# vibevoice-community/VibeVoice

Measured on NVIDIA H100. Metric: audio_seconds_per_second, higher is better.
Workload: dtype bf16

## Files before the change

### include/vibevoice_b200.h

```cpp
#ifndef VIBEVOICE_B200_H_
#define VIBEVOICE_B200_H_

#include <stdint.h>

#ifdef __cplusplus
extern "C" {
#endif

#define VV_ABI_VERSION 1

typedef struct vv_ctx vv_ctx;

typedef enum {
  VV_OK = 0,
  VV_ERR_INVALID = -1,
  VV_ERR_CUDA = -2,
  VV_ERR_STATE = -3,
  VV_ERR_NOMEM = -4
} vv_status;

typedef enum { VV_DT_BF16 = 0, VV_DT_F32 = 1, VV_DT_F16 = 2 } vv_dtype;

typedef struct {
  int32_t hidden_size, intermediate_size, num_layers, num_q_heads, num_kv_heads, head_dim, vocab_size;
  int32_t max_position_embeddings, tie_word_embeddings;
  float rms_norm_eps, rope_theta;
  int32_t head_layers, head_ffn_dim, latent_size;
  float head_rms_eps;
  int32_t n_stages;
  int32_t dec_ratios[8];
  int32_t dec_depths[8];
  int32_t dec_n_filters;
  int32_t enc_ratios[8];
  int32_t enc_depths[8];
  int32_t enc_n_filters;
  int32_t acoustic_vae_dim, semantic_vae_dim;
  float codec_eps;
  int32_t n_valid_ids;
  int32_t valid_ids[8];
  int32_t max_batch;
  int32_t max_diffusion_steps;
} vv_model_desc;

int vv_abi_version(void);
const char* vv_last_error(void);
int vv_create(const vv_model_desc* desc, int device, vv_ctx** out);
void vv_destroy(vv_ctx* ctx);

int vv_load_tensor(vv_ctx* ctx, const char* name, const void* data, int dtype, const int64_t* shape, int ndim);
int vv_set_speech_factors(vv_ctx* ctx, float scaling_factor, float bias_factor);
int vv_finalize_weights(vv_ctx* ctx);
int64_t vv_weight_bytes(vv_ctx* ctx, int which);

int vv_kv_init(vv_ctx* ctx, int64_t n_pages);
int vv_kv_reserve(vv_ctx* ctx, int seq, int64_t n_tokens, void* stream);
int vv_kv_set_len(vv_ctx* ctx, int seq, int64_t len, void* stream);
int vv_kv_write(vv_ctx* ctx, int seq, int layer, int64_t pos0, int64_t n_tokens,
                const void* k_bf16, const void* v_bf16, void* stream);
int vv_kv_delete_slot(vv_ctx* ctx, int seq, int64_t pos, void* stream);
int64_t vv_kv_pages_free(vv_ctx* ctx);
int64_t vv_kv_pages_total(vv_ctx* ctx);

int vv_set_rope_inv_freq(vv_ctx* ctx, const float* inv_freq_host, int n);
int vv_set_row_mode(vv_ctx* ctx, const int32_t* row_mode_host, void* stream);
int vv_lm_decode(vv_ctx* ctx, const float* embeds, float* hidden, float* logits, int32_t* tokens, void* stream);
int vv_lm_head(vv_ctx* ctx, const float* hidden , float* logits, int32_t* tokens, void* stream);
int vv_lm_logits_full(vv_ctx* ctx, const float* hidden , float* logits_out, void* stream);
int vv_lm_decode_range(vv_ctx* ctx, const float* embeds, int layer_begin, int layer_end, int final_norm, float* hidden, void* stream);
int vv_kv_commit(vv_ctx* ctx, const int32_t* advance_host, void* stream);
int64_t vv_kv_len(vv_ctx* ctx, int seq);
int vv_embed_tokens(vv_ctx* ctx, const int32_t* tokens_host, int n, float* out , void* stream);

int vv_set_diffusion_steps(vv_ctx* ctx, int n_steps, const float* timesteps, const float* coef, void* stream);
int vv_set_diffusion_steps_sde(vv_ctx* ctx, int n_steps, const float* timesteps, const float* coef7, void* stream);
int vv_set_step_noise(vv_ctx* ctx, const float* step_noise);
int vv_diffusion_sample(vv_ctx* ctx, const float* cond, const float* noise, const int32_t* active, float cfg_scale,
                        float* latent_out, void* stream);

int vv_codec_decode_frame(vv_ctx* ctx, const float* latent, const int32_t* active, float* audio_out , void* stream);
int vv_semantic_encode_frame(vv_ctx* ctx, const float* audio , const int32_t* active, float* feat_out , void* stream);
int vv_connect(vv_ctx* ctx, const float* latent , const float* sem , const int32_t* active,
               float* embeds_inout , void* stream);
int vv_codec_state_zero(vv_ctx* ctx, const int32_t* rows_host, int n, void* stream);
int vv_codec_state_reset(vv_ctx* ctx, void* stream);

int vv_frame_tail(vv_ctx* ctx, const float* hidden, const float* noise, const int32_t* active, float cfg_scale,
                  float* latent_out, float* audio_out, float* embeds_inout, void* stream);

int64_t vv_launch_count(vv_ctx* ctx);
int vv_debug_gemv(vv_ctx* ctx, const void* w_bf16, const float* bias, const float* x, float* y, int M, int N, int K,
                  int prologue, const float* pro_w, float eps, int epilogue, void* stream);

int vv_debug_barrier_bench(vv_ctx* ctx, int iters, int ctas_per_sm, float* ms_out);
int vv_debug_stream_gemv(vv_ctx* ctx, const void* w_bf16, const float* bias, const float* x, float* y, int M, int N, int K, int prologue,
                         const float* pro_w, float eps, int alpha_kind, const float* alpha, int accumulate, void* stream);
int vv_debug_stream_gemv2(vv_ctx* ctx, const void* w_bf16, const float* bias, const float* x, int64_t ldx, float* y, int64_t ldy, int M, int N,
                          int K, int prologue, const float* pro_w, float eps, const float* pro_shift, const float* pro_scale, int64_t pro_ld,
                          int alpha_kind, const float* alpha, int64_t lda, int store, int64_t operand_cap, void* stream);
int vv_stream_trace_read2(vv_ctx* ctx, long long* out , int max_ops);
int vv_stream_trace_read(vv_ctx* ctx, long long* out , int* out_meta , int max_ops, const char* program_prefix);
int vv_stream_diag(vv_ctx* ctx, unsigned* out6);

#ifdef __cplusplus
}
#endif
#endif
```

### vibevoice_b200/_native.py

```python
from __future__ import annotations

import ctypes as C
import os
from typing import Optional, Sequence

import numpy as np

_HERE = os.path.dirname(os.path.abspath(__file__))
LIB_PATH = os.path.join(_HERE, "csrc", "libvibevoice_b200.so")

VV_DT_BF16, VV_DT_F32, VV_DT_F16 = 0, 1, 2
PRO_NONE, PRO_RMSNORM, PRO_ADALN, PRO_SILU = 0, 1, 2, 3
EPI_NONE, EPI_RESID, EPI_GATED_RESID, EPI_GAMMA_RESID, EPI_SWIGLU, EPI_GELU, EPI_SILU = 0, 2, 3, 4, 5, 6, 7


class VVError(RuntimeError):
    pass


class ModelDesc(C.Structure):
    _fields_ = [
        ("hidden_size", C.c_int32), ("intermediate_size", C.c_int32), ("num_layers", C.c_int32),
        ("num_q_heads", C.c_int32), ("num_kv_heads", C.c_int32), ("head_dim", C.c_int32), ("vocab_size", C.c_int32),
        ("max_position_embeddings", C.c_int32), ("tie_word_embeddings", C.c_int32),
        ("rms_norm_eps", C.c_float), ("rope_theta", C.c_float),
        ("head_layers", C.c_int32), ("head_ffn_dim", C.c_int32), ("latent_size", C.c_int32), ("head_rms_eps", C.c_float),
        ("n_stages", C.c_int32), ("dec_ratios", C.c_int32 * 8), ("dec_depths", C.c_int32 * 8), ("dec_n_filters", C.c_int32),
        ("enc_ratios", C.c_int32 * 8), ("enc_depths", C.c_int32 * 8), ("enc_n_filters", C.c_int32),
        ("acoustic_vae_dim", C.c_int32), ("semantic_vae_dim", C.c_int32), ("codec_eps", C.c_float),
        ("n_valid_ids", C.c_int32), ("valid_ids", C.c_int32 * 8),
        ("max_batch", C.c_int32), ("max_diffusion_steps", C.c_int32),
    ]


_P, _I, _L, _F = C.c_void_p, C.c_int, C.c_int64, C.c_float
SYMBOLS = {
    "vv_abi_version": (_I, []),
    "vv_last_error": (C.c_char_p, []),
    "vv_create": (_I, [C.POINTER(ModelDesc), _I, C.POINTER(_P)]),
    "vv_destroy": (None, [_P]),
    "vv_load_tensor": (_I, [_P, C.c_char_p, _P, _I, C.POINTER(_L), _I]),
    "vv_set_speech_factors": (_I, [_P, _F, _F]),
    "vv_finalize_weights": (_I, [_P]),
    "vv_weight_bytes": (_L, [_P, _I]),
    "vv_kv_init": (_I, [_P, _L]),
    "vv_kv_reserve": (_I, [_P, _I, _L, _P]),
    "vv_kv_set_len": (_I, [_P, _I, _L, _P]),
    "vv_kv_write": (_I, [_P, _I, _I, _L, _L, _P, _P, _P]),
    "vv_kv_delete_slot": (_I, [_P, _I, _L, _P]),
    "vv_kv_pages_free": (_L, [_P]),
    "vv_kv_pages_total": (_L, [_P]),
    "vv_set_rope_inv_freq": (_I, [_P, _P, _I]),
    "vv_set_row_mode": (_I, [_P, _P, _P]),
    "vv_lm_decode": (_I, [_P, _P, _P, _P, _P, _P]),
    "vv_lm_head": (_I, [_P, _P, _P, _P, _P]),
    "vv_lm_logits_full": (_I, [_P, _P, _P, _P]),
    "vv_lm_decode_range": (_I, [_P, _P, _I, _I, _I, _P, _P]),
    "vv_kv_commit": (_I, [_P, _P, _P]),
    "vv_kv_len": (_L, [_P, _I]),
    "vv_embed_tokens": (_I, [_P, _P, _I, _P, _P]),
    "vv_set_diffusion_steps": (_I, [_P, _I, _P, _P, _P]),
    "vv_set_diffusion_steps_sde": (_I, [_P, _I, _P, _P, _P]),
    "vv_set_step_noise": (_I, [_P, _P]),
    "vv_diffusion_sample": (_I, [_P, _P, _P, _P, _F, _P, _P]),
    "vv_codec_decode_frame": (_I, [_P, _P, _P, _P, _P]),
    "vv_semantic_encode_frame": (_I, [_P, _P, _P, _P, _P]),
    "vv_connect": (_I, [_P, _P, _P, _P, _P, _P]),
    "vv_codec_state_zero": (_I, [_P, _P, _I, _P]),
    "vv_codec_state_reset": (_I, [_P, _P]),
    "vv_frame_tail": (_I, [_P, _P, _P, _P, _F, _P, _P, _P, _P]),
    "vv_launch_count": (_L, [_P]),
    "vv_debug_barrier_bench": (_I, [_P, _I, _I, C.POINTER(C.c_float)]),
    "vv_debug_gemv": (_I, [_P, _P, _P, _P, _P, _I, _I, _I, _I, _P, _F, _I, _P]),
    "vv_debug_stream_gemv": (_I, [_P, _P, _P, _P, _P, _I, _I, _I, _I, _P, _F, _I, _P, _I, _P]),
    "vv_debug_stream_gemv2": (_I, [_P, _P, _P, _P, _L, _P, _L, _I, _I, _I, _I, _P, _F, _P, _P, _L, _I, _P, _L, _I, _L, _P]),
    "vv_stream_diag": (_I, [_P, _P]),
    "vv_stream_trace_read": (_I, [_P, _P, _P, _I, C.c_char_p]),
    "vv_stream_trace_read2": (_I, [_P, _P, _I]),
}

_lib = None


def load_library(path: Optional[str] = None):
    global _lib
    if _lib is not None and path is None:
        return _lib
    p = path or LIB_PATH
    if not os.path.exists(p):
        raise VVError("libvibevoice_b200.so not built (%s). Run `python -c 'import __graft_entry__ as g; g.build()'`; "
                      "there is no CPU fallback." % p)
    lib = C.CDLL(p)
    for name, (res, args) in SYMBOLS.items():
        fn = getattr(lib, name)
        fn.restype, fn.argtypes = res, args
    if path is None:
        _lib = lib
    return lib


def check(rc: int, what: str = ""):
    if rc < 0:
        msg = load_library().vv_last_error().decode("utf-8", "replace")
        raise VVError("%s failed (%d): %s" % (what or "vibevoice_b200 call", rc, msg))
    return rc


def iptr(a: np.ndarray):
    return a.ctypes.data_as(C.c_void_p)


def i32(seq: Sequence[int]) -> np.ndarray:
    return np.ascontiguousarray(np.asarray(seq, dtype=np.int32))
```

### vibevoice_b200/csrc/vv_kernels.cuh

```cuda
#pragma once
#include <cuda_bf16.h>
#include <cuda_runtime.h>
#include <stdint.h>

#define VV_DEVINL __device__ __forceinline__

namespace vv {

typedef __nv_bfloat16 bf16;

enum Prologue { PRO_NONE = 0, PRO_RMSNORM = 1, PRO_ADALN = 2, PRO_SILU = 3 };
enum Epilogue { EPI_NONE = 0, EPI_RESID = 2, EPI_GATED_RESID = 3, EPI_GAMMA_RESID = 4, EPI_SWIGLU = 5, EPI_GELU = 6, EPI_SILU = 7 };

struct RowMap {
  int T;
  long long bs;
  long long rs;
  VV_DEVINL long long off(int m) const { return (long long)(m / T) * bs + (long long)(m % T) * rs; }
};

static inline RowMap dense_rows(long long ld) { RowMap r; r.T = 1 << 30; r.bs = 0; r.rs = ld; return r; }

struct GemvP {
  const bf16* W;
  const float* bias;
  const float* x;
  RowMap xmap;
  float* y;
  int ldy;
  int M, N, K;
  int pro;
  const float* pro_w;
  float pro_eps;
  const float* pro_shift;
  const float* pro_scale;
  long long pro_ld;
  int epi;
  const float* epi_a;
  long long epi_lda;
  const float* res;
  int ldres;
  int WK;
};

VV_DEVINL void pdl_trigger() { asm volatile("griddepcontrol.launch_dependents;" ::: "memory"); }
VV_DEVINL void pdl_wait() { asm volatile("griddepcontrol.wait;" ::: "memory"); }

VV_DEVINL float warp_sum(float v) {
#pragma unroll
  for (int o = 16; o > 0; o >>= 1) v += __shfl_xor_sync(0xffffffffu, v, o);
  return v;
}
VV_DEVINL float warp_max(float v) {
#pragma unroll
  for (int o = 16; o > 0; o >>= 1) v = fmaxf(v, __shfl_xor_sync(0xffffffffu, v, o));
  return v;
}
VV_DEVINL float silu_f(float x) { return x / (1.0f + __expf(-x)); }
VV_DEVINL float gelu_erf_f(float x) { return 0.5f * x * (1.0f + erff(x * 0.70710678118654752440f)); }

VV_DEVINL uint4 ldg_stream(const void* p) {
  uint4 r;
  asm volatile("ld.global.nc.L1::no_allocate.v4.u32 {%0,%1,%2,%3}, [%4];"
               : "=r"(r.x), "=r"(r.y), "=r"(r.z), "=r"(r.w) : "l"(p));
  return r;
}
VV_DEVINL void bf16x8_unpack(const uint4& u, float* f) {
  f[0] = __uint_as_float(u.x << 16); f[1] = __uint_as_float(u.x & 0xffff0000u);
  f[2] = __uint_as_float(u.y << 16); f[3] = __uint_as_float(u.y & 0xffff0000u);
  f[4] = __uint_as_float(u.z << 16); f[5] = __uint_as_float(u.z & 0xffff0000u);
  f[6] = __uint_as_float(u.w << 16); f[7] = __uint_as_float(u.w & 0xffff0000u);
}
VV_DEVINL float bf16_bits_to_f(unsigned short b) { return __uint_as_float(((unsigned)b) << 16); }

VV_DEVINL int xs_pos(int k) {
  int c = k >> 8, kk = k & 255;
  int lane = kk >> 3, j = kk & 7;
  return (c << 8) + ((j >> 2) << 7) + (lane << 2) + (j & 3);
}

VV_DEVINL void epi_store_e(const GemvP& p, int epi, int m, int n, float v) {
  switch (epi) {
    case EPI_RESID: v += p.res[(long long)m * p.ldres + n]; break;
    case EPI_GATED_RESID: v = p.res[(long long)m * p.ldres + n] + p.epi_a[(long long)m * p.epi_lda + n] * v; break;
    case EPI_GAMMA_RESID: v = p.res[(long long)m * p.ldres + n] + p.epi_a[n] * v; break;
    case EPI_GELU: v = gelu_erf_f(v); break;
    case EPI_SILU: v = silu_f(v); break;
    default: break;
  }
  p.y[(long long)m * p.ldy + n] = v;
}
VV_DEVINL void epi_store(const GemvP& p, int m, int n, float v) { epi_store_e(p, p.epi, m, n, v); }

template <int MB>
__global__ void __launch_bounds__(256) gemv_kernel(GemvP p) {
  extern __shared__ __align__(16) float smem_f[];
  const int K = p.K, N = p.N;
  const int Kp = (K + 255) & ~255;
  float* xs = smem_f;
  float* red = smem_f + MB * Kp;
  __shared__ float s_part[MB][8];
  const int tid = threadIdx.x, lane = tid & 31, warp = tid >> 5;
  const int WK = p.WK, WR = 8 / WK;
  const int wr = warp / WK, wk = warp % WK;
  const int ntasks = (N + 4 * WR - 1) / (4 * WR);
  const int nchunks = (K + 255) >> 8;
  const int klane = lane * 8;

  auto load_chunk = [&](uint4 (&wv)[4], const bf16* const (&wrow)[4], int c) {
    if (c < nchunks && (c << 8) + klane < K) {
#pragma unroll
      for (int r = 0; r < 4; ++r) wv[r] = ldg_stream(wrow[r] + (c << 8));
    } else {
#pragma unroll
      for (int r = 0; r < 4; ++r) wv[r] = make_uint4(0u, 0u, 0u, 0u);
    }
  };
  auto set_rows = [&](const bf16* (&wrow)[4], int task) {
    const int r0 = (task * WR + wr) * 4;
#pragma unroll
    for (int r = 0; r < 4; ++r) wrow[r] = p.W + (size_t)min(r0 + r, N - 1) * K + klane;
  };

  pdl_trigger();
  for (int m0 = 0; m0 < p.M; m0 += MB) {
    __syncthreads();
    int task = blockIdx.x;
    const bf16* wrow[4];
    uint4 cur[4], nxt[4];
    int c = wk;
    if (task < ntasks) {
      set_rows(wrow, task);
      load_chunk(cur, wrow, c);
      load_chunk(nxt, wrow, c + WK);
    }
    pdl_wait();
    const bool need_inv = (p.pro == PRO_RMSNORM || p.pro == PRO_ADALN);
    const int K4 = K >> 2;
    constexpr int XR = 4;
    const bool one_pass = (K4 <= XR * 256);
    for (int m = 0; m < MB; ++m) {
      const bool valid = (m0 + m < p.M);
      const float* xr = p.x + (valid ? p.xmap.off(m0 + m) : 0);
      float4 xv[XR];
      float inv = 1.f;
      if (need_inv) {
        float ss = 0.f;
        if (one_pass) {
#pragma unroll
          for (int i = 0; i < XR; ++i) {
            const int q = tid + i * 256;
            xv[i] = (valid && q < K4) ? *reinterpret_cast<const float4*>(xr + 4 * q) : make_float4(0.f, 0.f, 0.f, 0.f);
            ss += xv[i].x * xv[i].x + xv[i].y * xv[i].y + xv[i].z * xv[i].z + xv[i].w * xv[i].w;
          }
        } else if (valid) {
          for (int q = tid; q < K4; q += 256) { const float4 v = *reinterpret_cast<const float4*>(xr + 4 * q); ss += v.x * v.x + v.y * v.y + v.z * v.z + v.w * v.w; }
        }
        ss = warp_sum(ss);
        if (lane == 0) s_part[m][warp] = ss;
        __syncthreads();
        float t = 0.f;
#pragma unroll
        for (int i = 0; i < 8; ++i) t += s_part[m][i];
        inv = rsqrtf(t / (float)K + p.pro_eps);
      }
      auto xform_store = [&](int k, float4 v, bool have) {
        if (valid && k < K) {
          if (!have) v = *reinterpret_cast<const float4*>(xr + k);
          if (p.pro == PRO_RMSNORM) {
            const float4 w = *reinterpret_cast<const float4*>(p.pro_w + k);
            v.x *= inv * w.x; v.y *= inv * w.y; v.z *= inv * w.z; v.w *= inv * w.w;
          } else if (p.pro == PRO_ADALN) {
            float4 w = make_float4(1.f, 1.f, 1.f, 1.f);
            if (p.pro_w) w = *reinterpret_cast<const float4*>(p.pro_w + k);
            const long long o = (long long)(m0 + m) * p.pro_ld + k;
            const float4 sc = *reinterpret_cast<const float4*>(p.pro_scale + o);
            const float4 sh = *reinterpret_cast<const float4*>(p.pro_shift + o);
            v.x = v.x * inv * w.x * (1.f + sc.x) + sh.x; v.y = v.y * inv * w.y * (1.f + sc.y) + sh.y;
            v.z = v.z * inv * w.z * (1.f + sc.z) + sh.z; v.w = v.w * inv * w.w * (1.f + sc.w) + sh.w;
          } else if (p.pro == PRO_SILU) {
            v.x = silu_f(v.x); v.y = silu_f(v.y); v.z = silu_f(v.z); v.w = silu_f(v.w);
          }
        } else {
          v = make_float4(0.f, 0.f, 0.f, 0.f);
        }
        *reinterpret_cast<float4*>(xs + m * Kp + xs_pos(k)) = v;
      };
#pragma unroll
      for (int i = 0; i < XR; ++i) {
        const int q = tid + i * 256;
        if (q < (Kp >> 2)) xform_store(q << 2, xv[i], need_inv && one_pass);
      }
      for (int q = tid + XR * 256; q < (Kp >> 2); q += 256) xform_store(q << 2, make_float4(0.f, 0.f, 0.f, 0.f), false);
    }
    __syncthreads();
// ... 421 lines not shown
               : "+f"(d[0]), "+f"(d[1]), "+f"(d[2]), "+f"(d[3]), "+f"(d[4]), "+f"(d[5]), "+f"(d[6]), "+f"(d[7]), "+f"(d[8]), "+f"(d[9]), "+f"(d[10]), "+f"(d[11]), "+f"(d[12]), "+f"(d[13]), "+f"(d[14]), "+f"(d[15]), "+f"(d[16]), "+f"(d[17]), "+f"(d[18]), "+f"(d[19]), "+f"(d[20]), "+f"(d[21]), "+f"(d[22]), "+f"(d[23]), "+f"(d[24]), "+f"(d[25]), "+f"(d[26]), "+f"(d[27]), "+f"(d[28]), "+f"(d[29]), "+f"(d[30]), "+f"(d[31])
               : "l"(a), "l"(b), "r"(accumulate) : "memory");
}

__global__ void split_bf16_kernel(const float* __restrict__ x, RowMap xmap, bf16* __restrict__ hi, bf16* __restrict__ lo, int M, int K) {
  pdl_trigger();
  pdl_wait();
  const long long n4 = (long long)M * (K >> 2);
  for (long long i = (long long)blockIdx.x * blockDim.x + threadIdx.x; i < n4; i += (long long)gridDim.x * blockDim.x) {
    const int m = (int)(i / (K >> 2)), k = (int)(i % (K >> 2)) << 2;
    const float4 v = *reinterpret_cast<const float4*>(x + xmap.off(m) + k);
    const float h0 = __bfloat162float(__float2bfloat16_rn(v.x)), h1 = __bfloat162float(__float2bfloat16_rn(v.y));
    const float h2 = __bfloat162float(__float2bfloat16_rn(v.z)), h3 = __bfloat162float(__float2bfloat16_rn(v.w));
    *reinterpret_cast<uint2*>(hi + (size_t)m * K + k) = make_uint2(pack_bf16(h0, h1), pack_bf16(h2, h3));
    *reinterpret_cast<uint2*>(lo + (size_t)m * K + k) = make_uint2(pack_bf16(v.x - h0, v.y - h1), pack_bf16(v.z - h2, v.w - h3));
  }
}

__global__ void __launch_bounds__(128) gemm_wgmma_kernel(GemvP p, const bf16* __restrict__ a_hi, const bf16* __restrict__ a_lo) {
  extern __shared__ unsigned char wg_raw[];
  const unsigned raw_addr = smem_u32(wg_raw);
  unsigned char* sm = wg_raw + ((1024u - (raw_addr & 1023u)) & 1023u);
  const int tid = threadIdx.x, lane = tid & 31, warp = tid >> 5;
  const int bn = blockIdx.x * WG_BM;
  const int bm = blockIdx.y * WG_BN;
  const int K = p.K, nk = (K + WG_BK - 1) / WG_BK;

  auto load_w = [&](int stage, int kb) {
    unsigned char* wt = sm + stage * WG_STAGE;
#pragma unroll
    for (int i = 0; i < 8; ++i) {
      const int idx = tid + i * 128, r = idx >> 3, c = idx & 7;
      const int n = bn + r, k = kb * WG_BK + c * 8;
      const bool ok = (n < p.N) && (k < K);
      cp_async16(wt + r * 128 + ((c ^ (r & 7)) << 4), p.W + (size_t)(ok ? n : 0) * K + (ok ? k : 0), ok ? 16 : 0);
    }
  };
  auto load_a = [&](int stage, int kb) {
    unsigned char* ah = sm + stage * WG_STAGE + WG_BM * 128;
#pragma unroll
    for (int i = 0; i < 8; ++i) {
      const int idx = tid + i * 128, pl = idx >> 9, r = (idx >> 3) & 63, c = idx & 7;
      const int m = bm + r, k = kb * WG_BK + c * 8;
      const bool ok = (m < p.M) && (k < K);
      const bf16* src = (pl ? a_lo : a_hi) + (size_t)(ok ? m : 0) * K + (ok ? k : 0);
      cp_async16(ah + pl * (WG_BN * 128) + r * 128 + ((c ^ (r & 7)) << 4), src, ok ? 16 : 0);
    }
  };
  float acc[2][32];
#pragma unroll
  for (int h = 0; h < 2; ++h)
#pragma unroll
    for (int i = 0; i < 32; ++i) acc[h][i] = 0.f;

  pdl_trigger();
  load_w(0, 0);
  if (nk > 1) load_w(1, 1);
  pdl_wait();
  load_a(0, 0);
  cp_async_commit();
  if (nk > 1) load_a(1, 1);
  cp_async_commit();
  for (int kb = 0; kb < nk; ++kb) {
    const int st = kb % WG_NST;
    cp_async_wait<1>();
    asm volatile("fence.proxy.async.shared::cta;" ::: "memory");
    __syncthreads();
    const unsigned wbase = smem_u32(sm + st * WG_STAGE);
    const unsigned long long dw = wgmma_desc_sw128(wbase), dh = wgmma_desc_sw128(wbase + WG_BM * 128),
                             dl = wgmma_desc_sw128(wbase + WG_BM * 128 + WG_BN * 128);
    wgmma_fence();
#pragma unroll
    for (int k = 0; k < WG_BK / 16; ++k) {
#pragma unroll
      for (int h = 0; h < 2; ++h) {
        wgmma_m64n64(acc[h], dw + 512 * h + 2 * k, dh + 2 * k, 1);
        wgmma_m64n64(acc[h], dw + 512 * h + 2 * k, dl + 2 * k, 1);
      }
    }
    wgmma_commit();
    if (kb + 2 < nk) {
      wgmma_wait<1>();
      __syncthreads();
      load_w((kb + 2) % WG_NST, kb + 2);
      load_a((kb + 2) % WG_NST, kb + 2);
    }
    cp_async_commit();
  }
  wgmma_wait<0>();
#pragma unroll
  for (int h = 0; h < 2; ++h)
#pragma unroll
    for (int e = 0; e < 2; ++e) {
      const int n = bn + h * 64 + warp * 16 + (lane >> 2) + 8 * e;
      if (n >= p.N) continue;
      const float bias = p.bias ? p.bias[n] : 0.f;
#pragma unroll
      for (int j = 0; j < WG_BN / 8; ++j)
#pragma unroll
        for (int c = 0; c < 2; ++c) {
          const int m = bm + 8 * j + 2 * (lane & 3) + c;
          if (m < p.M) epi_store(p, m, n, acc[h][4 * j + 2 * e + c] + bias);
        }
    }
}

__global__ void conv_naive_kernel(const float* __restrict__ W, const float* __restrict__ bias, const float* __restrict__ x,
                                  RowMap xmap, float* __restrict__ y, int M, int N, int K) {
  pdl_trigger();
  pdl_wait();
  const long long idx = (long long)blockIdx.x * blockDim.x + threadIdx.x;
  if (idx >= (long long)M * N) return;
  const int m = (int)(idx / N), n = (int)(idx % N);
  const float* xr = x + xmap.off(m);
  const float* wr = W + (size_t)n * K;
  float acc = bias ? bias[n] : 0.f;
  for (int k = 0; k < K; ++k) acc = fmaf(wr[k], xr[k], acc);
  y[idx] = acc;
}

__global__ void __launch_bounds__(256) conv_warp_kernel(const float* __restrict__ W, const float* __restrict__ bias, const float* __restrict__ x,
                                                        RowMap xmap, float* __restrict__ y, int M, int N, int K) {
  pdl_trigger();
  pdl_wait();
  const long long idx = (long long)blockIdx.x * (blockDim.x >> 5) + (threadIdx.x >> 5);
  const int lane = threadIdx.x & 31;
  if (idx >= (long long)M * N) return;
  const int m = (int)(idx / N), n = (int)(idx % N);
  const float* xr = x + xmap.off(m);
  const float* wr = W + (size_t)n * K;
  float acc = 0.f;
  for (int k = lane; k < K; k += 32) acc = fmaf(wr[k], xr[k], acc);
  acc = warp_sum(acc);
  if (lane == 0) y[idx] = acc + (bias ? bias[n] : 0.f);
}

__global__ void rows_norm_kernel(const float* __restrict__ x, const float* __restrict__ w, float* __restrict__ y,
                                 int M, int C, float eps) {
  pdl_trigger();
  pdl_wait();
  const int row = blockIdx.x * (blockDim.x >> 5) + (threadIdx.x >> 5);
  const int lane = threadIdx.x & 31;
  if (row >= M) return;
  const float* xr = x + (size_t)row * C;
  float ss = 0.f;
  for (int c = lane; c < C; c += 32) { float v = xr[c]; ss += v * v; }
  ss = warp_sum(ss);
  const float inv = rsqrtf(ss / (float)C + eps);
  for (int c = lane; c < C; c += 32) y[(size_t)row * C + c] = xr[c] * inv * (w ? w[c] : 1.f);
}

__global__ void assemble_window_kernel(const float* __restrict__ src, const float* __restrict__ hist,
                                       float* __restrict__ win, float* __restrict__ hist_next, int B, int T, int ctx, int C,
                                       const float* __restrict__ norm_w, float eps, float alpha, float beta) {
  pdl_trigger();
  pdl_wait();
  const int row = blockIdx.x * (blockDim.x >> 5) + (threadIdx.x >> 5);
  const int lane = threadIdx.x & 31;
  const int R = ctx + T;
  if (row >= B * R) return;
  const int b = row / R, j = row % R;
  float* wr = win + ((size_t)b * R + j) * C;
  float* hn = (j >= T) ? hist_next + ((size_t)b * ctx + (j - T)) * C : nullptr;
  if (j < ctx) {
    const float* hr = hist + ((size_t)b * ctx + j) * C;
    for (int c = lane; c < C; c += 32) { float v = hr[c]; wr[c] = v; if (hn) hn[c] = v; }
  } else {
    const float* sr = src + ((size_t)b * T + (j - ctx)) * C;
    float inv = 1.f;
    if (norm_w) {
      float ss = 0.f;
      for (int c = lane; c < C; c += 32) { float v = sr[c]; ss += v * v; }
      ss = warp_sum(ss);
      inv = rsqrtf(ss / (float)C + eps);
    }
    for (int c = lane; c < C; c += 32) {
      float v = norm_w ? sr[c] * inv * norm_w[c] : sr[c] * alpha + beta;
      wr[c] = v;
      if (hn) hn[c] = v;
    }
  }
}

__global__ void __launch_bounds__(256) assemble_window_block_kernel(const float* __restrict__ src, const float* __restrict__ hist,
                                                                    float* __restrict__ win, float* __restrict__ hist_next, int B, int T,
                                                                    int ctx, int C, const float* __restrict__ norm_w, float eps, float alpha,
                                                                    float beta) {
  pdl_trigger();
  pdl_wait();
  const int row = blockIdx.x, tid = threadIdx.x;
  const int R = ctx + T;
  const int b = row / R, j = row % R;
  float* wr = win + ((size_t)b * R + j) * C;
  float* hn = (j >= T) ? hist_next + ((size_t)b * ctx + (j - T)) * C : nullptr;
  __shared__ float sp[8];
  if (j < ctx) {
    const float* hr = hist + ((size_t)b * ctx + j) * C;
    for (int c = tid; c < C; c += 256) { float v = hr[c]; wr[c] = v; if (hn) hn[c] = v; }
  } else {
    const float* sr = src + ((size_t)b * T + (j - ctx)) * C;
    float inv = 1.f;
    if (norm_w) {
      float ss = 0.f;
      for (int c = tid; c < C; c += 256) { float v = sr[c]; ss += v * v; }
      ss = warp_sum(ss);
      if ((tid & 31) == 0) sp[tid >> 5] = ss;
      __syncthreads();
      float t = 0.f;
#pragma unroll
      for (int i = 0; i < 8; ++i) t += sp[i];
      inv = rsqrtf(t / (float)C + eps);
    }
    for (int c = tid; c < C; c += 256) {
      float v = norm_w ? sr[c] * inv * norm_w[c] : sr[c] * alpha + beta;
      wr[c] = v;
      if (hn) hn[c] = v;
    }
  }
}
__global__ void __launch_bounds__(256) rows_norm_block_kernel(const float* __restrict__ x, const float* __restrict__ w, float* __restrict__ y,
                                                              int C, float eps) {
  pdl_trigger();
  pdl_wait();
  const int row = blockIdx.x, tid = threadIdx.x;
  const float* xr = x + (size_t)row * C;
  __shared__ float sp[8];
  float ss = 0.f;
  for (int c = tid; c < C; c += 256) { float v = xr[c]; ss += v * v; }
  ss = warp_sum(ss);
  if ((tid & 31) == 0) sp[tid >> 5] = ss;
  __syncthreads();
  float t = 0.f;
#pragma unroll
  for (int i = 0; i < 8; ++i) t += sp[i];
  const float inv = rsqrtf(t / (float)C + eps);
  for (int c = tid; c < C; c += 256) y[(size_t)row * C + c] = xr[c] * inv * (w ? w[c] : 1.f);
}

__global__ void dwconv_res_kernel(const float* __restrict__ x, const float* __restrict__ win, const float* __restrict__ w ,
                                  const float* __restrict__ bias, const float* __restrict__ gamma, float* __restrict__ out,
                                  int B, int T, int C) {
  pdl_trigger();
  pdl_wait();
  const long long idx = (long long)blockIdx.x * blockDim.x + threadIdx.x;
  if (idx >= (long long)B * T * C) return;
  const int c = (int)(idx % C);
  const long long bt = idx / C;
  const int t = (int)(bt % T), b = (int)(bt / T);
  const float* wp = win + ((size_t)b * (T + 6) + t) * C + c;
  float acc = bias[c];
#pragma unroll
  for (int j = 0; j < 7; ++j) acc = fmaf(w[j * C + c], wp[(size_t)j * C], acc);
  out[idx] = x[idx] + gamma[c] * acc;
}

struct StateSeg { float* hist; float* next; int n; };

constexpr int ADV_SLICES = 8;
__global__ void advance_kernel(const StateSeg* __restrict__ segs, const int* __restrict__ active) {
  pdl_trigger();
  pdl_wait();
  const int b = blockIdx.y;
  if (active && !active[b]) return;
  const StateSeg s = segs[blockIdx.x];
  float* d = s.hist + (size_t)b * s.n;
  const float* a = s.next + (size_t)b * s.n;
  for (int i = blockIdx.z * blockDim.x + threadIdx.x; i < s.n; i += gridDim.z * blockDim.x) d[i] = a[i];
}
__global__ void state_zero_kernel(const StateSeg* __restrict__ segs, const int* __restrict__ rows) {
  const int b = rows[blockIdx.y];
  const StateSeg s = segs[blockIdx.x];
  float* d = s.hist + (size_t)b * s.n;
  for (int i = threadIdx.x; i < s.n; i += blockDim.x) d[i] = 0.f;
}

constexpr int KV_PAGE = 64;
constexpr int HD = 128;

struct KvView {
  bf16* kpool; bf16* vpool;
  const int* page_table;
  int max_pages;
  const int* kv_len;
  const int* row_mode;
  int kv_heads, q_heads;
};

__global__ void rope_append_kernel(const float* __restrict__ qkv, float* __restrict__ q_rot, KvView kv,
                                   const float* __restrict__ inv_freq ) {
  pdl_trigger();
  pdl_wait();
  const int m = blockIdx.x;
  if (!kv.row_mode[m]) return;
  const int pos = kv.kv_len[m];
  const int nq = kv.q_heads, nkv = kv.kv_heads;
  const float* row = qkv + (size_t)m * (nq + 2 * nkv) * HD;
  const int page = kv.page_table[(size_t)m * kv.max_pages + pos / KV_PAGE];
  const int slot = pos % KV_PAGE;
  for (int i = threadIdx.x; i < (nq + nkv) * (HD / 2); i += blockDim.x) {
    const int h = i / (HD / 2), d = i % (HD / 2);
    const float ang = (float)pos * inv_freq[d];
    float sn, cs;
    sincosf(ang, &sn, &cs);
    const float x1 = row[h * HD + d], x2 = row[h * HD + d + HD / 2];
    const float o1 = x1 * cs - x2 * sn, o2 = x2 * cs + x1 * sn;
    if (h < nq) {
      q_rot[((size_t)m * nq + h) * HD + d] = o1;
      q_rot[((size_t)m * nq + h) * HD + d + HD / 2] = o2;
    } else {
      bf16* kp = kv.kpool + (((size_t)page * nkv + (h - nq)) * KV_PAGE + slot) * HD;
      kp[d] = __float2bfloat16_rn(o1);
      kp[d + HD / 2] = __float2bfloat16_rn(o2);
    }
  }
  for (int i = threadIdx.x; i < nkv * HD; i += blockDim.x) {
    const int h = i / HD, d = i % HD;
    bf16* vp = kv.vpool + (((size_t)page * nkv + h) * KV_PAGE + slot) * HD;
    vp[d] = __float2bfloat16_rn(row[(nq + nkv + h) * HD + d]);
  }
}

constexpr int ATT_TILE = 32;
constexpr int ATT_MAXG = 8;
__global__ void __launch_bounds__(128) attn_partial_kernel(const float* __restrict__ q_rot, KvView kv, float* __restrict__ part_acc,
                                                           float* __restrict__ part_ml, int nsplit, float scale) {
  pdl_trigger();
  pdl_wait();
  const int s = blockIdx.x, g = blockIdx.y, m = blockIdx.z;
  if (!kv.row_mode[m]) return;
  const int G = kv.q_heads / kv.kv_heads;
  const int L = kv.kv_len[m] + 1;
  const int ntiles = (L + ATT_TILE - 1) / ATT_TILE;
  const int tps = (ntiles + nsplit - 1) / nsplit;
  const int t_begin = s * tps, t_end = min(ntiles, (s + 1) * tps);
  const int tid = threadIdx.x, lane = tid & 31, warp = tid >> 5;

  __shared__ __align__(16) bf16 Ks[2][ATT_TILE][HD + 8];
  __shared__ __align__(16) bf16 Vs[2][ATT_TILE][HD + 8];
  __shared__ __align__(16) float qs[ATT_MAXG][HD];
  __shared__ float ps[ATT_MAXG][ATT_TILE];

  auto prefetch = [&](int t, int buf) {
    const int tok0 = t * ATT_TILE;
    const int page = kv.page_table[(size_t)m * kv.max_pages + tok0 / KV_PAGE];
    const size_t base = (((size_t)page * kv.kv_heads + g) * KV_PAGE + (tok0 % KV_PAGE)) * HD;
#pragma unroll
    for (int it = 0; it < 4; ++it) {
      const int idx = tid + it * 128;
      const int r = idx >> 4, c = (idx & 15) * 8;
      cp_async16(&Ks[buf][r][c], kv.kpool + base + (size_t)r * HD + c, 16);
      cp_async16(&Vs[buf][r][c], kv.vpool + base + (size_t)r * HD + c, (tok0 + r < L) ? 16 : 0);
    }
  };
  if (t_begin < t_end) prefetch(t_begin, 0);
  cp_async_commit();
  for (int i = tid; i < G * HD; i += 128) qs[i / HD][i % HD] = q_rot[((size_t)m * kv.q_heads + g * G) * HD + i];

  float m_run[2] = {-INFINITY, -INFINITY}, l_run[2] = {0.f, 0.f};
  float acc[2][4] = {{0.f, 0.f, 0.f, 0.f}, {0.f, 0.f, 0.f, 0.f}};

  for (int t = t_begin; t < t_end; ++t) {
    const int buf = (t - t_begin) & 1;
    const int tok0 = t * ATT_TILE;
    if (t + 1 < t_end) prefetch(t + 1, buf ^ 1);
    cp_async_commit();
    cp_async_wait<1>();
    __syncthreads();
#pragma unroll
    for (int hh = 0; hh < 2; ++hh) {
      const int h = warp + 4 * hh;
      if (h >= G) continue;
      float sc = 0.f;
#pragma unroll
      for (int c = 0; c < HD; c += 8) {
        float kf[8];
        bf16x8_unpack(*reinterpret_cast<const uint4*>(&Ks[buf][lane][c]), kf);
        const float4 qa = *reinterpret_cast<const float4*>(&qs[h][c]);
        const float4 qb = *reinterpret_cast<const float4*>(&qs[h][c + 4]);
        sc = fmaf(kf[0], qa.x, sc); sc = fmaf(kf[1], qa.y, sc); sc = fmaf(kf[2], qa.z, sc); sc = fmaf(kf[3], qa.w, sc);
        sc = fmaf(kf[4], qb.x, sc); sc = fmaf(kf[5], qb.y, sc); sc = fmaf(kf[6], qb.z, sc); sc = fmaf(kf[7], qb.w, sc);
      }
      sc = (tok0 + lane < L) ? sc * scale : -INFINITY;
      const float mt = warp_max(sc);
      const float mn = fmaxf(m_run[hh], mt);
      const float pj = __expf(sc - mn);
      const float corr = __expf(m_run[hh] - mn);
      l_run[hh] = l_run[hh] * corr + warp_sum(pj);
      m_run[hh] = mn;
      ps[h][lane] = pj;
      __syncwarp();
#pragma unroll
      for (int j = 0; j < 4; ++j) acc[hh][j] *= corr;
#pragma unroll 8
      for (int tt = 0; tt < ATT_TILE; ++tt) {
        const float pv = ps[h][tt];
        const uint2 v2 = *reinterpret_cast<const uint2*>(&Vs[buf][tt][lane * 4]);
        acc[hh][0] = fmaf(pv, __uint_as_float(v2.x << 16), acc[hh][0]);
        acc[hh][1] = fmaf(pv, __uint_as_float(v2.x & 0xffff0000u), acc[hh][1]);
        acc[hh][2] = fmaf(pv, __uint_as_float(v2.y << 16), acc[hh][2]);
        acc[hh][3] = fmaf(pv, __uint_as_float(v2.y & 0xffff0000u), acc[hh][3]);
      }
      __syncwarp();
    }
    __syncthreads();
  }
#pragma unroll
// ... 434 lines not shown
```

### vibevoice_b200/csrc/vv_runtime.cu

```cuda
#include "../../include/vibevoice_b200.h"
#include "vv_kernels.cuh"
#include "vv_stream.cuh"

#include <cuda.h>
#include <cuda_fp16.h>

#include <algorithm>
#include <initializer_list>
#include <cmath>
#include <cstdarg>
#include <cstdio>
#include <cstdlib>
#include <cstring>
#include <map>
#include <set>
#include <string>
#include <tuple>
#include <vector>

using namespace vv;

static thread_local std::string g_err;
static int fail(int code, const char* fmt, ...) {
  char buf[2048];
  va_list ap;
  va_start(ap, fmt);
  vsnprintf(buf, sizeof buf, fmt, ap);
  va_end(ap);
  g_err = buf;
  return code;
}
#define CK(expr)                                                                                     \
  do {                                                                                               \
    cudaError_t _e = (expr);                                                                         \
    if (_e != cudaSuccess) return fail(VV_ERR_CUDA, "%s:%d %s -> %s", __FILE__, __LINE__, #expr, cudaGetErrorString(_e)); \
  } while (0)
#define CKL() CK(cudaGetLastError())
#define RET(expr)            \
  do {                       \
    int _r = (expr);         \
    if (_r < 0) return _r;   \
  } while (0)

struct RawTensor {
  void* p = nullptr;
  std::vector<int64_t> shape;
  bool is_f32 = false;
  size_t numel = 0;
};

struct Block {
  int C = 0;
  float *norm_w = nullptr, *dw_w = nullptr, *dw_b = nullptr, *gamma = nullptr, *ffn_norm_w = nullptr, *b1 = nullptr, *b2 = nullptr,
        *ffn_gamma = nullptr;
  bf16 *w1 = nullptr, *w2 = nullptr;
  float *hist = nullptr, *next = nullptr;
};
struct ConvL {
  int Cin = 0, Cout = 0, k = 0, stride = 1, ctx = 0, N = 0, K = 0;
  bf16* w = nullptr; float* wf = nullptr; float* bias = nullptr;
  float *hist = nullptr, *next = nullptr;
};
struct Codec {
  std::vector<ConvL> convs;
  std::vector<std::vector<Block>> stages;
  std::vector<int> T;
  std::vector<int> C;
  StateSeg* segs_dev = nullptr; int n_segs = 0;
  int64_t weight_bytes = 0;
};
struct LmLayer { bf16 *wqkv, *wo, *wgu, *wdown; float *bqkv, *ln1, *ln2; };
struct HeadLayer { bf16 *wgu, *wdown; float* norm; };

struct GraphEntry { cudaGraphExec_t exec = nullptr; int64_t launches = 0; };

struct vv_ctx {
  vv_model_desc d;
  int device = 0;
  bool finalized = false;
  bool use_graphs = true;
  bool use_pdl = true;
  bool use_mma_attn = true;
  bool use_splitk = true;
  bool fuse_rope = true;
  bf16* s_planes = nullptr; size_t planes_elems = 0;
  int mma_min_rows = 9;
  int use_wgmma = 1;
  bool ring_rms = true;
  int codec_mma_min_rows = 9;
  bool mma_ring = true;
  bf16* head_slab = nullptr; size_t head_slab_bytes = 0; size_t l2_persist_bytes = 0; size_t l2_window_max = 0;
  int wr_tasks_min = 296;
  int wr_force = 0;
  int gemv_grid_cap = 0;
  int sm_count = 132;
  std::map<std::string, RawTensor> raw;
  std::set<std::string> expected;
  std::vector<void*> allocs;
  float speech_scale = NAN, speech_bias = NAN;
  std::vector<LmLayer> lm;
  float* lm_norm = nullptr; bf16* embed = nullptr; const bf16* lm_head_w = nullptr; bf16* head_valid = nullptr; int* valid_ids_dev = nullptr; float* inv_freq = nullptr;
  int Nqkv = 0;
  bf16 *h_noisy = nullptr, *h_cond = nullptr, *h_t0 = nullptr, *h_t2 = nullptr, *h_mod = nullptr, *h_final = nullptr;
  std::vector<HeadLayer> head;
  int n_steps = 0; float* temb = nullptr; DpmCoef* coef_dev = nullptr; float* tfreqs = nullptr;
  std::vector<DpmCoef> coef_host; int coef_version = 0;
  bool sde = false; const float* step_noise = nullptr;
  bf16 *ca_fc1 = nullptr, *ca_fc2 = nullptr, *cs_fc1 = nullptr, *cs_fc2 = nullptr;
  float *ca_b1 = nullptr, *ca_b2 = nullptr, *ca_n = nullptr, *cs_b1 = nullptr, *cs_b2 = nullptr, *cs_n = nullptr;
  Codec dec, enc;
  int64_t wbytes[6] = {0, 0, 0, 0, 0, 0};
  int64_t n_pages = 0; int max_pages = 0; bf16 *kpool = nullptr, *vpool = nullptr;
  int* page_table_dev = nullptr; int* kv_len_dev = nullptr; int* row_mode_dev = nullptr;
  std::vector<int64_t> kv_len_host; std::vector<std::vector<int>> seq_pages; std::vector<int> free_pages;
  float* s_lgu = nullptr;
  float *s_h = nullptr, *s_qkv = nullptr, *s_qrot = nullptr, *s_attn = nullptr, *s_act = nullptr, *s_pacc = nullptr, *s_pml = nullptr;
  int nsplit = 128;
  float *s_condp = nullptr, *s_call = nullptr, *s_mod = nullptr, *s_hx = nullptr, *s_hg = nullptr, *s_v = nullptr, *s_z = nullptr,
        *s_x0 = nullptr, *s_tfeat = nullptr, *s_t1 = nullptr, *s_hgu = nullptr;
  float *s_xa = nullptr, *s_xb = nullptr, *s_u = nullptr, *s_win = nullptr, *s_xn = nullptr;
  float *s_e = nullptr, *s_c1 = nullptr, *s_feat = nullptr, *s_audio = nullptr, *s_latent = nullptr;
  int* s_tok = nullptr;
  std::map<std::string, GraphEntry> graphs;
  GridBar* gridbar = nullptr;
  struct StreamProg {
    SOp* ops = nullptr; int n_ops = 0; CUtensorMap* tmaps = nullptr; int n_stages = 0; int b_bytes = 0; int smem = 0; int gemv_ops = 0; int variant = 0;
    std::vector<int> op_first;
  };
  std::map<std::string, StreamProg> sprogs;
  unsigned* st_bar = nullptr;
  unsigned* st_diag_host = nullptr; unsigned* st_diag_dev = nullptr;
  int st_inflight = 4;
  float* dec_front_x = nullptr;
  float *s_cx = nullptr, *s_cu = nullptr;
  int use_stream = 15;
  float* s_rope = nullptr;
  float *s_pacc2 = nullptr, *s_pml2 = nullptr;
  std::map<std::tuple<const bf16*, int, int>, bf16*> tiled; size_t tiled_bytes = 0;
  long long* st_trace2 = nullptr;
  long long* st_trace = nullptr; int st_trace_ops = 0; int st_trace_cta = 0; int st_trace_last_ops = 0;
  float* cfg_dev = nullptr; float cfg_last = NAN;
  int64_t launches = 0;
  std::map<long long, int> occ_cache;
};

struct L {
  vv_ctx* c; cudaStream_t s;
  const void* win_base = nullptr;
  size_t win_bytes = 0;
  float win_ratio = 0.f;
};

template <typename... KArgs, typename... Args>
static cudaError_t launch_k(const L& l, void (*kern)(KArgs...), dim3 grid, dim3 block, size_t smem, Args... args) {
  cudaLaunchConfig_t cfg;
  memset(&cfg, 0, sizeof cfg);
  cfg.gridDim = grid; cfg.blockDim = block; cfg.dynamicSmemBytes = smem; cfg.stream = l.s;
  cudaLaunchAttribute attr[2];
  int na = 0;
  if (l.c->use_pdl) {
    attr[na].id = cudaLaunchAttributeProgrammaticStreamSerialization;
    attr[na].val.programmaticStreamSerializationAllowed = 1;
    ++na;
  }
  if (l.win_bytes) {
    attr[na].id = cudaLaunchAttributeAccessPolicyWindow;
    attr[na].val.accessPolicyWindow.base_ptr = const_cast<void*>(l.win_base);
    attr[na].val.accessPolicyWindow.num_bytes = l.win_bytes;
    attr[na].val.accessPolicyWindow.hitRatio = l.win_ratio;
    attr[na].val.accessPolicyWindow.hitProp = cudaAccessPropertyPersisting;
    attr[na].val.accessPolicyWindow.missProp = cudaAccessPropertyStreaming;
    ++na;
  }
  cfg.attrs = attr;
  cfg.numAttrs = na;
  l.c->launches++;
  return cudaLaunchKernelEx(&cfg, kern, KArgs(args)...);
}

template <class T>
static int dmalloc(vv_ctx* c, T** p, size_t n, bool zero = true) {
  void* q = nullptr;
  cudaError_t e = cudaMalloc(&q, std::max<size_t>(n, 1) * sizeof(T));
  if (e != cudaSuccess) return fail(VV_ERR_NOMEM, "cudaMalloc(%zu bytes): %s", n * sizeof(T), cudaGetErrorString(e));
  if (zero) cudaMemset(q, 0, std::max<size_t>(n, 1) * sizeof(T));
  c->allocs.push_back(q);
  *p = (T*)q;
  return 0;
}

static int gemv_smem_bytes(int MB, int K) { int Kp = (K + 255) & ~255; return (MB * Kp + 2 * 8 * 4 * MB) * 4; }

template <int MB>
static int launch_gemv_t(const L& l, GemvP& p, int grid, int smem) {
  static bool attr_set[8] = {false, false, false, false, false, false, false, false};
  (void)attr_set;
  CK(cudaFuncSetAttribute(gemv_kernel<MB>, cudaFuncAttributeMaxDynamicSharedMemorySize, 200 * 1024));
  CK(launch_k(l, gemv_kernel<MB>, dim3(grid), dim3(256), smem, p));
  return 0;
}

template <int MB>
static int gemv_occupancy(vv_ctx* c, int smem) {
  long long key = ((long long)MB << 32) | (unsigned)smem;
  auto it = c->occ_cache.find(key);
  if (it != c->occ_cache.end()) return it->second;
  int occ = 1;
  cudaFuncSetAttribute(gemv_kernel<MB>, cudaFuncAttributeMaxDynamicSharedMemorySize, 200 * 1024);
  if (cudaOccupancyMaxActiveBlocksPerMultiprocessor(&occ, gemv_kernel<MB>, 256, smem) != cudaSuccess || occ < 1) occ = 1;
  c->occ_cache[key] = occ;
  return occ;
}

static int linear(const L& l, GemvP p) {
  if (p.K % 8 != 0) return fail(VV_ERR_INVALID, "linear: K=%d not a multiple of 8", p.K);
  if (((uintptr_t)p.x & 15) || (p.xmap.rs & 3) || (p.xmap.bs & 3)) return fail(VV_ERR_INVALID, "linear: activation rows must be 16-byte aligned");
  const int wg_ctas = ((p.N + WG_BM - 1) / WG_BM) * ((p.M + WG_BN - 1) / WG_BN);
  if (l.c->use_wgmma && p.M > 8 && p.pro == PRO_NONE && p.epi != EPI_SWIGLU && (l.c->use_wgmma == 2 || wg_ctas >= 96)) {
    if ((size_t)p.M * p.K > l.c->planes_elems) return fail(VV_ERR_INVALID, "wgmma: activation planes scratch too small (%d x %d)", p.M, p.K);
    bf16* hi = l.c->s_planes;
    bf16* lo = l.c->s_planes + l.c->planes_elems;
    const long long n4 = (long long)p.M * (p.K >> 2);
    CK(launch_k(l, split_bf16_kernel, dim3((unsigned)std::min<long long>((n4 + 255) / 256, 1184)), dim3(256), 0, p.x, p.xmap, hi, lo, p.M, p.K));
    CK(cudaFuncSetAttribute(gemm_wgmma_kernel, cudaFuncAttributeMaxDynamicSharedMemorySize, WG_SMEM));
    CK(launch_k(l, gemm_wgmma_kernel, dim3((p.N + WG_BM - 1) / WG_BM, (p.M + WG_BN - 1) / WG_BN), dim3(128), (size_t)WG_SMEM, p, (const bf16*)hi, (const bf16*)lo));
    return 0;
  }
  if (p.M >= l.c->mma_min_rows) {
    dim3 grid((p.N + MM_BN - 1) / MM_BN, (p.M + MM_BM - 1) / MM_BM);
    const bool inplace_res = (p.epi == EPI_RESID || p.epi == EPI_GAMMA_RESID || p.epi == EPI_GATED_RESID) && p.res == p.y && p.ldres == p.ldy;
    const int nk = (p.K + MM_BK - 1) / MM_BK;
    if (l.c->use_splitk && inplace_res && nk >= 8 && (int)(grid.x * grid.y) < l.c->sm_count) {
      int z = std::min(std::min(nk / 2, 16), (2 * l.c->sm_count) / (int)(grid.x * grid.y));
      grid.z = std::max(z, 1);
    }
    const bool ring_rms = p.pro == PRO_RMSNORM && grid.z == 1 && p.K <= MR_MAXK_NORM && p.K % 4 == 0;
    if (l.c->mma_ring && (p.pro == PRO_NONE || ring_rms) && p.epi != EPI_SWIGLU) {
      void (*fn)(GemvP) = gemm_mma_ring_kernel<-1, -1>;
      if (!getenv("VV_RING_GENERIC")) {
        if (ring_rms && p.epi == EPI_GELU) fn = gemm_mma_ring_kernel<1, EPI_GELU>;
        else if (ring_rms && p.epi == EPI_NONE) fn = gemm_mma_ring_kernel<1, EPI_NONE>;
        else if (!ring_rms && p.epi == EPI_GAMMA_RESID) fn = gemm_mma_ring_kernel<0, EPI_GAMMA_RESID>;
        else if (!ring_rms && p.epi == EPI_NONE) fn = gemm_mma_ring_kernel<0, EPI_NONE>;
        else if (!ring_rms && p.epi == EPI_GELU) fn = gemm_mma_ring_kernel<0, EPI_GELU>;
        else if (!ring_rms && p.epi == EPI_RESID) fn = gemm_mma_ring_kernel<0, EPI_RESID>;
      }
      CK(cudaFuncSetAttribute(fn, cudaFuncAttributeMaxDynamicSharedMemorySize, MR_SMEM_NORM));
      CK(launch_k(l, fn, dim3(grid), dim3(128), (size_t)(ring_rms ? MR_SMEM_NORM : MR_SMEM), p));
      return 0;
    }
    CK(launch_k(l, gemm_mma_kernel, dim3(grid), dim3(128), 0, p));
    return 0;
  }
  int MB = p.M <= 1 ? 1 : (p.M <= 2 ? 2 : (p.M <= 4 ? 4 : 8));
  while (MB > 1 && gemv_smem_bytes(MB, p.K) > 200 * 1024) MB >>= 1;
  if (gemv_smem_bytes(MB, p.K) > 200 * 1024) return fail(VV_ERR_INVALID, "gemv: K=%d too large", p.K);
  int WR = 8;
  while (WR > 1 && (p.N + 4 * WR - 1) / (4 * WR) < l.c->wr_tasks_min) WR >>= 1;
  const int nchunks = (p.K + 255) / 256;
  while (WR < 8 && 8 / WR > nchunks) WR <<= 1;
  if (l.c->wr_force) WR = l.c->wr_force;
  p.WK = 8 / WR;
  const int ntasks = (p.N + 4 * WR - 1) / (4 * WR);
  const int smem = gemv_smem_bytes(MB, p.K);
  int occ = MB == 1 ? gemv_occupancy<1>(l.c, smem) : MB == 2 ? gemv_occupancy<2>(l.c, smem) : MB == 4 ? gemv_occupancy<4>(l.c, smem)
                                                                                                          : gemv_occupancy<8>(l.c, smem);
  int grid = std::min(ntasks, l.c->sm_count * occ);
  if (l.c->gemv_grid_cap) grid = std::min(grid, l.c->gemv_grid_cap);
  switch (MB) {
    case 1: return launch_gemv_t<1>(l, p, grid, smem);
    case 2: return launch_gemv_t<2>(l, p, grid, smem);
    case 4: return launch_gemv_t<4>(l, p, grid, smem);
    default: return launch_gemv_t<8>(l, p, grid, smem);
  }
}

static GemvP mk(const bf16* W, const float* bias, const float* x, long long ldx, float* y, int ldy, int M, int N, int K) {
  GemvP p;
  memset(&p, 0, sizeof p);
  p.W = W; p.bias = bias; p.x = x; p.xmap = dense_rows(ldx); p.y = y; p.ldy = ldy; p.M = M; p.N = N; p.K = K;
  p.pro = PRO_NONE; p.epi = EPI_NONE; p.WK = 1;
  return p;
}

typedef CUresult (*EncodeTiledFn)(CUtensorMap*, CUtensorMapDataType, cuuint32_t, void*, const cuuint64_t*, const cuuint64_t*, const cuuint32_t*,
                                  const cuuint32_t*, CUtensorMapInterleave, CUtensorMapSwizzle, CUtensorMapL2promotion, CUtensorMapFloatOOBfill);
static EncodeTiledFn encode_tiled_fn() {
  static EncodeTiledFn fn = nullptr;
  if (!fn) {
    void* p = nullptr;
    cudaDriverEntryPointQueryResult q;
    if (cudaGetDriverEntryPoint("cuTensorMapEncodeTiled", &p, cudaEnableDefault, &q) == cudaSuccess && q == cudaDriverEntryPointSuccess) fn = (EncodeTiledFn)p;
  }
  return fn;
}
static int make_weight_tmap(const bf16* T, long long n_tiles, CUtensorMap* out) {
  EncodeTiledFn enc = encode_tiled_fn();
  if (!enc) return fail(VV_ERR_CUDA, "cuTensorMapEncodeTiled is not available from this driver");
  const int N = (int)n_tiles, K = 64;
  const cuuint64_t dims[2] = {64, (cuuint64_t)n_tiles * 128};
  const cuuint64_t strides[1] = {128};
  const cuuint32_t box[2] = {64, 128};
  const cuuint32_t estr[2] = {1, 1};
  CUresult r = enc(out, CU_TENSOR_MAP_DATA_TYPE_BFLOAT16, 2, (void*)T, dims, strides, box, estr, CU_TENSOR_MAP_INTERLEAVE_NONE,
                   CU_TENSOR_MAP_SWIZZLE_128B, CU_TENSOR_MAP_L2_PROMOTION_NONE, CU_TENSOR_MAP_FLOAT_OOB_FILL_NONE);
  if (r != CUDA_SUCCESS) return fail(VV_ERR_CUDA, "cuTensorMapEncodeTiled([%d tiles x %d]) failed with %d", N, K, (int)r);
  return 0;
}
static int tiled_weight(vv_ctx* c, const bf16* W, long long ldw, int N, int K, int k0, bool fresh, bf16** out, long long* n_tiles) {
  if (K % 8 || k0 % 8 || ldw % 8 || ((uintptr_t)W & 15))
    return fail(VV_ERR_INVALID, "stream: weight [%d x %d] must have K %% 8 == 0 and a 16-byte aligned base", N, K);
  const long long KB = (K + 63) / 64, R = (N + 127) / 128;
  *n_tiles = R * KB;
  const auto key = std::make_tuple(W, k0, K);
  if (!fresh) {
    auto it = c->tiled.find(key);
    if (it != c->tiled.end()) { *out = it->second; return 0; }
  }
  bf16* T = nullptr;
  RET(dmalloc(c, &T, (size_t)(*n_tiles) * 8192, false));
  const long long n_chunks = *n_tiles * 1024;
  tile_pack_kernel<<<(unsigned)std::min<long long>((n_chunks + 255) / 256, (long long)c->sm_count * 32), 256>>>(W, T, N, K, (int)KB, ldw, k0, n_chunks);
  CKL();
  CK(cudaDeviceSynchronize());
  if (!fresh) c->tiled[key] = T;
  c->tiled_bytes += (size_t)(*n_tiles) * 16384;
  *out = T;
  return 0;
}

struct StreamBuilder {
  vv_ctx* c;
  std::vector<SOp> ops;
  std::vector<CUtensorMap> tmaps;
  std::vector<const bf16*> wsrc;
  explicit StreamBuilder(vv_ctx* c_) : c(c_) {}
  SOp& push(int kind, bool sync) {
    SOp o;
    memset(&o, 0, sizeof o);
    o.kind = kind; o.sync_before = sync ? 1 : 0; o.nB = 16;
    ops.push_back(o); wsrc.push_back(nullptr);
    return ops.back();
  }
  bool fresh_weights = false;
  std::vector<bf16*> owned;
  long long operand_cap = 0;
  int kv_tmap = -1;
  std::vector<int> needs_kv;
  int use_kv_pool() {
    if (kv_tmap >= 0) return 0;
    const auto& d = c->d;
    EncodeTiledFn enc = encode_tiled_fn();
    if (!enc) return fail(VV_ERR_CUDA, "cuTensorMapEncodeTiled is not available from this driver");
    const cuuint64_t rows = (cuuint64_t)d.num_layers * c->n_pages * d.num_kv_heads * KV_PAGE;
    const cuuint64_t dims[2] = {(cuuint64_t)d.head_dim, rows};
    const cuuint64_t strides[1] = {(cuuint64_t)d.head_dim * 2};
    const cuuint32_t box[2] = {64, KV_PAGE};
    const cuuint32_t estr[2] = {1, 1};
    for (bf16* pool : {c->kpool, c->vpool}) {
      CUtensorMap tm;
      CUresult r = enc(&tm, CU_TENSOR_MAP_DATA_TYPE_BFLOAT16, 2, (void*)pool, dims, strides, box, estr, CU_TENSOR_MAP_INTERLEAVE_NONE,
                       CU_TENSOR_MAP_SWIZZLE_128B, CU_TENSOR_MAP_L2_PROMOTION_NONE, CU_TENSOR_MAP_FLOAT_OOB_FILL_NONE);
      if (r != CUDA_SUCCESS) return fail(VV_ERR_CUDA, "cuTensorMapEncodeTiled(KV pool) failed with %d", (int)r);
      tmaps.push_back(tm);
    }
    kv_tmap = (int)tmaps.size() - 2;
    return 0;
  }
  void fill_att(SAtt* a, int layer) {
    const auto& d = c->d;
    const size_t per_layer = (size_t)c->n_pages * d.num_kv_heads * KV_PAGE * d.head_dim;
    memset(a, 0, sizeof *a);
    a->hd = d.head_dim;
    a->qkv = c->s_qkv;
    a->kv.kpool = c->kpool + per_layer * layer; a->kv.vpool = c->vpool + per_layer * layer;
    a->kv.page_table = c->page_table_dev; a->kv.max_pages = c->max_pages; a->kv.kv_len = c->kv_len_dev; a->kv.row_mode = c->row_mode_dev;
    a->kv.kv_heads = d.num_kv_heads; a->kv.q_heads = d.num_q_heads;
    a->part_acc = c->s_pacc2; a->part_ml = c->s_pml2; a->inv_freq = c->inv_freq; a->scale = 1.0f / sqrtf((float)d.head_dim);
    a->row_base = (unsigned)((size_t)layer * c->n_pages * d.num_kv_heads * KV_PAGE);
    a->rope_cs = c->s_rope;
  }
  int attn(int layer, int M) {
    RET(use_kv_pool());
    SOp& o = push(SK_ATTN, true);
    o.M = M;
    fill_att(&o.att, layer);
    needs_kv.push_back((int)ops.size() - 1);
    return 0;
  }
  int gemv(const bf16* W, const float* bias, const float* x, long long ldx, float* y, long long ldy, int M, int N, int K, bool sync, SOp** out) {
    if (M < 1 || M > 32) return fail(VV_ERR_INVALID, "stream gemv: M=%d outside [1,32]", M);
    if (N < 1 || K < 8 || K % 8 || ((uintptr_t)W & 15))
      return fail(VV_ERR_INVALID, "stream: weight [%d x %d] must have K %% 8 == 0 and a 16-byte aligned base", N, K);
    SOp& o = push(SK_GEMV, sync);
    o.M = M; o.N = N; o.K = K; o.krow = K; o.nB = M <= 8 ? 16 : (M <= 16 ? 32 : 64);
    o.x = x; o.ldx = ldx; o.y = y; o.ldy = ldy; o.bias = bias; o.pro = SP_NONE; o.alpha_kind = SA_ONE;
    wsrc.back() = W;
// ... 121 lines not shown
  int b_bytes = 2048;
  for (const SOp& o : b.ops) {
    if (o.kind == SK_MIX && (o.cod.T_out > 8 || o.K % 4 || o.K > 4096)) return fail(VV_ERR_INVALID, "stream: mixer stage handles T <= 8, C <= 4096");
    if (o.kind == SK_ATTN) b_bytes = std::max(b_bytes, 32768);
    if (o.kind != SK_GEMV) continue;
    const long long KB = (o.K + 63) / 64, R = (o.N + 127) / 128, U = R * KB;
    const long long per = (U + G - 1) / G;
    long long nh;
    b_bytes = std::max<long long>(b_bytes, stage_operand_bytes(c, o, KB, &nh));
    const long long segs = (per + KB - 1) / KB + 1;
    if (segs > ST_MAXSEG) return fail(VV_ERR_INVALID, "stream: stage [%d x %d] needs %lld accumulators per CTA", o.N, o.K, segs);
    if (o.store && KB != 1) return fail(VV_ERR_INVALID, "stream: store epilogue needs K <= 64");
    if (o.pro == SP_WINDOW && (o.cod.cin % 8)) return fail(VV_ERR_INVALID, "stream: window prologue needs a channel count that is a multiple of 8");
    if (o.pro == SP_COMBINE) {
      const int hd = c->d.head_dim;
      if ((long long)o.M * nh > 128 || o.k0 % hd || o.K % hd || o.k0 + o.K > hd * c->d.num_q_heads)
        return fail(VV_ERR_INVALID, "stream: attention-merge prologue does not fit (M=%d, heads %d..%d, %lld per CTA)", o.M, o.k0 / hd,
                    (o.k0 + o.K) / hd, nh);
    }
    if (U * (G + 1) >= (1ll << 32)) return fail(VV_ERR_INVALID, "stream: stage [%d x %d] has too many tiles for 32-bit scheduling", o.N, o.K);
  }
  int ns = (max_dyn - 1024 - b_bytes) / ST_TILE;
  ns = std::min(ns, ST_MAX_STAGES);
  if (getenv("VV_STREAM_STAGES")) ns = std::min(ns, atoi(getenv("VV_STREAM_STAGES")));
  if (ns < 2) return fail(VV_ERR_INVALID, "stream: activation operand of %d bytes leaves no room for the weight ring", b_bytes);
  pr->n_stages = ns; pr->b_bytes = b_bytes; pr->smem = ns * ST_TILE + b_bytes + 1024;
  pr->n_ops = (int)b.ops.size();
  RET(dmalloc(c, &pr->tmaps, std::max<size_t>(b.tmaps.size(), 1), false));
  RET(dmalloc(c, &pr->ops, b.ops.size(), false));
  for (int i : b.needs_kv) {
    b.ops[i].att.tmap_k = (unsigned long long)(uintptr_t)(pr->tmaps + b.kv_tmap);
    b.ops[i].att.tmap_v = (unsigned long long)(uintptr_t)(pr->tmaps + b.kv_tmap + 1);
  }
  for (size_t i = 0; i < b.ops.size(); ++i) {
    if (tmap_of[i] >= 0) b.ops[i].tmap = (unsigned long long)(uintptr_t)(pr->tmaps + tmap_of[i]);
    pr->gemv_ops += b.ops[i].kind == SK_GEMV;
  }
  if (!b.tmaps.empty()) CK(cudaMemcpy(pr->tmaps, b.tmaps.data(), b.tmaps.size() * sizeof(CUtensorMap), cudaMemcpyHostToDevice));
  CK(cudaMemcpy(pr->ops, b.ops.data(), b.ops.size() * sizeof(SOp), cudaMemcpyHostToDevice));
  CK(cudaFuncSetAttribute(STREAM_VARIANTS[pr->variant].fn, cudaFuncAttributeMaxDynamicSharedMemorySize, max_dyn));
  CK(cudaFuncSetAttribute(STREAM_VARIANTS[pr->variant].fn_trace, cudaFuncAttributeMaxDynamicSharedMemorySize, max_dyn));
  return 0;
}

static int launch_stream(const L& l, const vv_ctx::StreamProg& pr, int op_begin = 0, int op_count = -1) {
  vv_ctx* c = l.c;
  const int n_built = (int)pr.op_first.size() - 1;
  if (op_count < 0) op_count = n_built - op_begin;
  if (op_begin < 0 || op_begin + op_count > n_built) return fail(VV_ERR_INVALID, "stream: stages [%d, +%d) outside the program", op_begin, op_count);
  const int op_end = pr.op_first[op_begin + op_count];
  op_begin = pr.op_first[op_begin];
  op_count = op_end - op_begin;
  CK(cudaMemsetAsync(c->st_bar, 0, sizeof(unsigned), l.s));
  cudaLaunchConfig_t cfg;
  memset(&cfg, 0, sizeof cfg);
  cfg.gridDim = dim3(c->sm_count); cfg.blockDim = dim3(ST_THREADS); cfg.dynamicSmemBytes = pr.smem; cfg.stream = l.s;
  cudaLaunchAttribute attr[1];
  attr[0].id = cudaLaunchAttributeCooperative;
  attr[0].val.cooperative = 1;
  cfg.attrs = attr; cfg.numAttrs = 1;
  SParams P;
  P.ops = pr.ops + op_begin; P.n_ops = op_count; P.bar_count = c->st_bar; P.diag = c->st_diag_dev; P.n_stages = pr.n_stages; P.b_bytes = pr.b_bytes;
  P.max_inflight = std::max(1, std::min(pr.n_stages, c->st_inflight));
  P.kv_len = c->kv_len_dev; P.row_mode = c->row_mode_dev; P.n_seq = 2 * c->d.max_batch; P.kv_heads = c->d.num_kv_heads;
  P.trace = (c->st_trace && op_count == pr.n_ops && pr.n_ops <= c->st_trace_ops) ? c->st_trace : nullptr; P.trace_cta = c->st_trace_cta;
  P.trace2 = P.trace ? c->st_trace2 : nullptr;
  if (P.trace) c->st_trace_last_ops = pr.n_ops;
  c->launches++;
  CK(cudaLaunchKernelEx(&cfg, P.trace ? STREAM_VARIANTS[pr.variant].fn_trace : STREAM_VARIANTS[pr.variant].fn, P));
  return 0;
}

static std::string S(const char* fmt, ...) {
  char buf[512];
  va_list ap;
  va_start(ap, fmt);
  vsnprintf(buf, sizeof buf, fmt, ap);
  va_end(ap);
  return buf;
}
static void block_names(std::set<std::string>& e, const std::string& p) {
  for (const char* s : {"norm.weight", "mixer.conv.conv.conv.weight", "mixer.conv.conv.conv.bias", "gamma", "ffn_norm.weight",
                        "ffn.linear1.weight", "ffn.linear1.bias", "ffn.linear2.weight", "ffn.linear2.bias", "ffn_gamma"})
    e.insert(p + "." + s);
}
static void build_expected(vv_ctx* c) {
  auto& e = c->expected;
  const auto& d = c->d;
  const std::string lm = "model.language_model";
  e.insert(lm + ".embed_tokens.weight");
  e.insert(lm + ".norm.weight");
  for (int l = 0; l < d.num_layers; ++l) {
    std::string q = S("%s.layers.%d", lm.c_str(), l);
    for (const char* s : {"self_attn.q_proj.weight", "self_attn.q_proj.bias", "self_attn.k_proj.weight", "self_attn.k_proj.bias",
                          "self_attn.v_proj.weight", "self_attn.v_proj.bias", "self_attn.o_proj.weight", "mlp.gate_proj.weight",
                          "mlp.up_proj.weight", "mlp.down_proj.weight", "input_layernorm.weight", "post_attention_layernorm.weight"})
      e.insert(q + "." + s);
  }
  if (!d.tie_word_embeddings) e.insert("lm_head.weight");
  const std::string h = "model.prediction_head";
  for (const char* s : {"noisy_images_proj.weight", "cond_proj.weight", "t_embedder.mlp.0.weight", "t_embedder.mlp.2.weight",
                        "final_layer.linear.weight", "final_layer.adaLN_modulation.1.weight"})
    e.insert(h + "." + s);
  for (int l = 0; l < d.head_layers; ++l)
    for (const char* s : {"ffn.gate_proj.weight", "ffn.up_proj.weight", "ffn.down_proj.weight", "norm.weight", "adaLN_modulation.1.weight"})
      e.insert(S("%s.layers.%d.%s", h.c_str(), l, s));
  for (const char* cn : {"model.acoustic_connector", "model.semantic_connector"})
    for (const char* s : {"fc1.weight", "fc1.bias", "norm.weight", "fc2.weight", "fc2.bias"}) e.insert(std::string(cn) + "." + s);
  const std::string dp = "model.acoustic_tokenizer.decoder", ep = "model.semantic_tokenizer.encoder";
  for (int i = 0; i < d.n_stages; ++i) {
    if (i == 0) { e.insert(dp + ".upsample_layers.0.0.conv.conv.weight"); e.insert(dp + ".upsample_layers.0.0.conv.conv.bias"); }
    else { e.insert(S("%s.upsample_layers.%d.0.convtr.convtr.weight", dp.c_str(), i)); e.insert(S("%s.upsample_layers.%d.0.convtr.convtr.bias", dp.c_str(), i)); }
    for (int j = 0; j < d.dec_depths[i]; ++j) block_names(e, S("%s.stages.%d.%d", dp.c_str(), i, j));
    e.insert(S("%s.downsample_layers.%d.0.conv.conv.weight", ep.c_str(), i));
    e.insert(S("%s.downsample_layers.%d.0.conv.conv.bias", ep.c_str(), i));
    for (int j = 0; j < d.enc_depths[i]; ++j) block_names(e, S("%s.stages.%d.%d", ep.c_str(), i, j));
  }
  for (const char* s : {"head.conv.conv.weight", "head.conv.conv.bias"}) { e.insert(dp + "." + s); e.insert(ep + "." + s); }
}

extern "C" int vv_abi_version(void) { return VV_ABI_VERSION; }
extern "C" const char* vv_last_error(void) { return g_err.c_str(); }

extern "C" int vv_create(const vv_model_desc* desc, int device, vv_ctx** out) {
  if (!desc || !out) return fail(VV_ERR_INVALID, "vv_create: null argument");
  if (desc->head_dim != 128 && desc->head_dim != 64) return fail(VV_ERR_INVALID, "head_dim %d unsupported (64 or 128)", desc->head_dim);
  if (desc->max_batch < 1 || desc->max_batch > 8) return fail(VV_ERR_INVALID, "max_batch must be in [1,8]");
  if (desc->n_stages < 2 || desc->n_stages > 8) return fail(VV_ERR_INVALID, "n_stages out of range");
  if (desc->num_q_heads % desc->num_kv_heads || desc->num_q_heads / desc->num_kv_heads > ATT_MAXG)
    return fail(VV_ERR_INVALID, "GQA group size unsupported");
  if (desc->latent_size != 64 || desc->acoustic_vae_dim != 64) return fail(VV_ERR_INVALID, "latent size must be 64");
  if (desc->n_valid_ids < 1 || desc->n_valid_ids > 8) return fail(VV_ERR_INVALID, "n_valid_ids out of range");
  CK(cudaSetDevice(device));
  vv_ctx* c = new vv_ctx();
  c->d = *desc;
  c->device = device;
  cudaDeviceProp prop;
  CK(cudaGetDeviceProperties(&prop, device));
  c->sm_count = prop.multiProcessorCount;
  const char* ng = getenv("VV_NO_GRAPH");
  c->use_graphs = !(ng && ng[0] == '1');
  const char* na = getenv("VV_SCALAR_ATTN");
  c->use_mma_attn = !(na && na[0] == '1');
  c->wr_tasks_min = c->sm_count;
  if (getenv("VV_WR_TASKS_MIN")) c->wr_tasks_min = atoi(getenv("VV_WR_TASKS_MIN"));
  if (getenv("VV_WR_FORCE")) c->wr_force = atoi(getenv("VV_WR_FORCE"));
  if (getenv("VV_GEMV_GRID_CAP")) c->gemv_grid_cap = atoi(getenv("VV_GEMV_GRID_CAP"));
  if (getenv("VV_NO_FUSE_ROPE")) c->fuse_rope = false;
  if (getenv("VV_STREAM")) c->use_stream = atoi(getenv("VV_STREAM"));
  if (getenv("VV_STREAM_INFLIGHT")) c->st_inflight = atoi(getenv("VV_STREAM_INFLIGHT"));
  if (getenv("VV_WGMMA")) c->use_wgmma = atoi(getenv("VV_WGMMA"));
  if (getenv("VV_MMA_MIN_ROWS")) c->mma_min_rows = atoi(getenv("VV_MMA_MIN_ROWS"));
  if (getenv("VV_NO_MMA_RING")) c->mma_ring = false;
  if (getenv("VV_NO_RING_RMS")) c->ring_rms = false;
  if (getenv("VV_CODEC_MMA_MIN_ROWS")) c->codec_mma_min_rows = atoi(getenv("VV_CODEC_MMA_MIN_ROWS"));
  else if (getenv("VV_MMA_MIN_ROWS")) c->codec_mma_min_rows = c->mma_min_rows;
  const char* ns = getenv("VV_NO_SPLITK");
  c->use_splitk = !(ns && ns[0] == '1');
  const char* np = getenv("VV_NO_PDL");
  c->use_pdl = !(np && np[0] == '1');
  build_expected(c);
  *out = c;
  return 0;
}

extern "C" void vv_destroy(vv_ctx* c) {
  if (!c) return;
  cudaSetDevice(c->device);
  cudaDeviceSynchronize();
  for (auto& g : c->graphs) if (g.second.exec) cudaGraphExecDestroy(g.second.exec);
  for (auto& r : c->raw) if (r.second.p) cudaFree(r.second.p);
  for (void* p : c->allocs) cudaFree(p);
  if (c->st_diag_host) cudaFreeHost(c->st_diag_host);
  delete c;
}

static bool stored_as_f32(const std::string& name, const int64_t* shape, int ndim) {
  if (ndim <= 1) return true;
  if (name.find("mixer.conv.conv.conv.weight") != std::string::npos) return true;
  if (ndim == 3 && (shape[0] == 1 || shape[1] == 1)) return true;
  return false;
}

extern "C" int vv_load_tensor(vv_ctx* c, const char* name_, const void* data, int dtype, const int64_t* shape, int ndim) {
  if (!c || !name_ || !data) return fail(VV_ERR_INVALID, "vv_load_tensor: null argument");
  if (c->finalized) return fail(VV_ERR_STATE, "vv_load_tensor after vv_finalize_weights");
  std::string name(name_);
  CK(cudaSetDevice(c->device));
  if (name == "model.speech_scaling_factor" || name == "model.speech_bias_factor") {
    float v; char tmp[4];
    CK(cudaMemcpy(tmp, data, dtype == VV_DT_F32 ? 4 : 2, cudaMemcpyDefault));
    if (dtype == VV_DT_F32) memcpy(&v, tmp, 4);
    else if (dtype == VV_DT_BF16) { unsigned u = ((unsigned)(*(unsigned short*)tmp)) << 16; memcpy(&v, &u, 4); }
    else v = __half2float(*(__half*)tmp);
    (name == "model.speech_scaling_factor" ? c->speech_scale : c->speech_bias) = v;
    return 0;
  }
  if (!c->expected.count(name)) {
    if (name.rfind("model.acoustic_tokenizer.encoder.", 0) == 0 || name.find("fix_std") != std::string::npos ||
        name.find("rotary_emb") != std::string::npos || (name == "lm_head.weight" && c->d.tie_word_embeddings))
      return 1;
    return fail(VV_ERR_INVALID, "vv_load_tensor: unknown tensor '%s'", name.c_str());
  }
  size_t n = 1;
  for (int i = 0; i < ndim; ++i) n *= (size_t)shape[i];
  RawTensor t;
  t.shape.assign(shape, shape + ndim);
  t.numel = n;
  t.is_f32 = stored_as_f32(name, shape, ndim);
  const size_t esz = dtype == VV_DT_F32 ? 4 : 2;
  void* dst = nullptr;
  CK(cudaMalloc(&dst, n * (t.is_f32 ? 4 : 2)));
  t.p = dst;
  const bool same = (t.is_f32 && dtype == VV_DT_F32) || (!t.is_f32 && dtype == VV_DT_BF16);
  if (same) {
    CK(cudaMemcpy(dst, data, n * esz, cudaMemcpyDefault));
  } else {
    void* tmp = nullptr;
    CK(cudaMalloc(&tmp, n * esz));
    CK(cudaMemcpy(tmp, data, n * esz, cudaMemcpyDefault));
    const int grid = (int)std::min<size_t>((n + 255) / 256, 65535);
    if (t.is_f32 && dtype == VV_DT_BF16) cvt_bf16_to_f32_kernel<<<grid, 256>>>((const bf16*)tmp, (float*)dst, n);
    else if (t.is_f32 && dtype == VV_DT_F16) cvt_f16_to_f32_kernel<<<grid, 256>>>((const __half*)tmp, (float*)dst, n);
    else if (!t.is_f32 && dtype == VV_DT_F32) cvt_f32_to_bf16_kernel<<<grid, 256>>>((const float*)tmp, (bf16*)dst, n);
    else cvt_f16_to_bf16_kernel<<<grid, 256>>>((const __half*)tmp, (bf16*)dst, n);
    CKL();
    CK(cudaDeviceSynchronize());
    cudaFree(tmp);
  }
  auto it = c->raw.find(name);
  if (it != c->raw.end() && it->second.p) cudaFree(it->second.p);
  c->raw[name] = t;
  return 0;
}

extern "C" int vv_set_speech_factors(vv_ctx* c, float s, float b) {
  if (!c) return fail(VV_ERR_INVALID, "null ctx");
  c->speech_scale = s; c->speech_bias = b;
  return 0;
}

static int need(vv_ctx* c, const std::string& name, RawTensor** t, std::vector<int64_t> shape) {
  auto it = c->raw.find(name);
  if (it == c->raw.end()) return fail(VV_ERR_STATE, "missing tensor %s", name.c_str());
  if (it->second.shape != shape) {
    std::string a, b;
    for (auto v : it->second.shape) a += std::to_string(v) + ",";
    for (auto v : shape) b += std::to_string(v) + ",";
    return fail(VV_ERR_INVALID, "tensor %s has shape [%s] expected [%s]", name.c_str(), a.c_str(), b.c_str());
  }
  *t = &it->second;
  return 0;
}
static int take_bf16(vv_ctx* c, const std::string& name, std::vector<int64_t> shape, bf16** out, int64_t* bytes) {
  RawTensor* t;
  RET(need(c, name, &t, shape));
  if (t->is_f32) return fail(VV_ERR_INVALID, "%s stored as f32, expected bf16", name.c_str());
  *out = (bf16*)t->p;
  c->allocs.push_back(t->p);
  t->p = nullptr;
  if (bytes) *bytes += (int64_t)t->numel * 2;
  return 0;
}
static int take_f32(vv_ctx* c, const std::string& name, std::vector<int64_t> shape, float** out, int64_t* bytes) {
  RawTensor* t;
  RET(need(c, name, &t, shape));
  if (!t->is_f32) return fail(VV_ERR_INVALID, "%s stored as bf16, expected f32", name.c_str());
  *out = (float*)t->p;
  c->allocs.push_back(t->p);
  t->p = nullptr;
  if (bytes) *bytes += (int64_t)t->numel * 2;
  return 0;
}
static void drop(vv_ctx* c, const std::string& name) {
  auto it = c->raw.find(name);
  if (it != c->raw.end() && it->second.p) { cudaFree(it->second.p); it->second.p = nullptr; }
}

static int build_block(vv_ctx* c, const std::string& p, int C, Block* b, int64_t* bytes, std::vector<StateSeg>* segs) {
  b->C = C;
  RET(take_f32(c, p + ".norm.weight", {C}, &b->norm_w, bytes));
  RawTensor* t;
  RET(need(c, p + ".mixer.conv.conv.conv.weight", &t, {C, 1, 7}));
  RET(dmalloc(c, &b->dw_w, (size_t)7 * C));
  repack_dw_kernel<<<(C * 7 + 255) / 256, 256>>>((const float*)t->p, b->dw_w, C);
  CKL();
  *bytes += (int64_t)C * 7 * 2;
  RET(take_f32(c, p + ".mixer.conv.conv.conv.bias", {C}, &b->dw_b, bytes));
  RET(take_f32(c, p + ".gamma", {C}, &b->gamma, bytes));
  RET(take_f32(c, p + ".ffn_norm.weight", {C}, &b->ffn_norm_w, bytes));
  RET(take_bf16(c, p + ".ffn.linear1.weight", {4 * C, C}, &b->w1, bytes));
  RET(take_f32(c, p + ".ffn.linear1.bias", {4 * C}, &b->b1, bytes));
  RET(take_bf16(c, p + ".ffn.linear2.weight", {C, 4 * C}, &b->w2, bytes));
  RET(take_f32(c, p + ".ffn.linear2.bias", {C}, &b->b2, bytes));
  RET(take_f32(c, p + ".ffn_gamma", {C}, &b->ffn_gamma, bytes));
  const int B = c->d.max_batch;
  RET(dmalloc(c, &b->hist, (size_t)B * 6 * C));
  RET(dmalloc(c, &b->next, (size_t)B * 6 * C));
  segs->push_back({b->hist, b->next, 6 * C});
  return 0;
}

static int build_conv(vv_ctx* c, const std::string& p, int Ci, int Co, int k, int stride, ConvL* L_, int64_t* bytes,
                      std::vector<StateSeg>* segs) {
  L_->Cin = Ci; L_->Cout = Co; L_->k = k; L_->stride = stride; L_->ctx = (k - 1) - (stride - 1); L_->N = Co; L_->K = k * Ci;
  RawTensor* t;
  RET(need(c, p + ".weight", &t, {Co, Ci, k}));
  const size_t n = (size_t)Co * Ci * k;
  if (t->is_f32) {
// ... 126 lines not shown
    RET(take_bf16(c, h + ".final_layer.linear.weight", {64, H}, &c->h_final, hb));
    const size_t modrows = (size_t)(3 * LH + 2) * H;
    RET(dmalloc(c, &c->h_mod, modrows * H, false));
    c->head.resize(LH);
    const size_t per_layer_el = (size_t)3 * F * H;
    c->head_slab_bytes = per_layer_el * LH * 2;
    RET(dmalloc(c, &c->head_slab, per_layer_el * LH, false));
    for (int l = 0; l < LH; ++l) {
      std::string q = S("%s.layers.%d", h.c_str(), l);
      RawTensor *tg, *tu, *tm, *td;
      RET(need(c, q + ".ffn.gate_proj.weight", &tg, {F, H}));
      RET(need(c, q + ".ffn.up_proj.weight", &tu, {F, H}));
      c->head[l].wgu = c->head_slab + per_layer_el * l;
      c->head[l].wdown = c->head[l].wgu + (size_t)2 * F * H;
      interleave_rows_kernel<<<4096, 256>>>((const bf16*)tg->p, (const bf16*)tu->p, c->head[l].wgu, (size_t)F, (size_t)H);
      CKL();
      CK(cudaDeviceSynchronize());
      *hb += (int64_t)2 * F * H * 2;
      drop(c, q + ".ffn.gate_proj.weight"); drop(c, q + ".ffn.up_proj.weight");
      RET(need(c, q + ".ffn.down_proj.weight", &td, {H, F}));
      CK(cudaMemcpy(c->head[l].wdown, td->p, (size_t)H * F * 2, cudaMemcpyDeviceToDevice));
      *hb += (int64_t)H * F * 2;
      drop(c, q + ".ffn.down_proj.weight");
      RET(take_f32(c, q + ".norm.weight", {H}, &c->head[l].norm, hb));
      RET(need(c, q + ".adaLN_modulation.1.weight", &tm, {3 * H, H}));
      CK(cudaMemcpy(c->h_mod + (size_t)l * 3 * H * H, tm->p, (size_t)3 * H * H * 2, cudaMemcpyDeviceToDevice));
      *hb += (int64_t)3 * H * H * 2;
      drop(c, q + ".adaLN_modulation.1.weight");
    }
    {
      int maxp = 0, maxw = 0;
      cudaDeviceGetAttribute(&maxp, cudaDevAttrMaxPersistingL2CacheSize, c->device);
      cudaDeviceGetAttribute(&maxw, cudaDevAttrMaxAccessPolicyWindowSize, c->device);
      size_t want = 0;
      if (getenv("VV_L2_PERSIST_MB")) want = (size_t)atoi(getenv("VV_L2_PERSIST_MB")) << 20;
      c->l2_persist_bytes = std::min<size_t>(want, (size_t)maxp);
      c->l2_window_max = (size_t)maxw;
      if (c->l2_persist_bytes) CK(cudaDeviceSetLimit(cudaLimitPersistingL2CacheSize, c->l2_persist_bytes));
      if (getenv("VV_VERBOSE")) fprintf(stderr, "[vv] L2 persisting max %d MB, window max %d MB, using %zu MB for a %zu MB head slab\n", maxp >> 20,
                                        maxw >> 20, c->l2_persist_bytes >> 20, c->head_slab_bytes >> 20);
    }
    RawTensor* tm;
    RET(need(c, h + ".final_layer.adaLN_modulation.1.weight", &tm, {2 * H, H}));
    CK(cudaMemcpy(c->h_mod + (size_t)LH * 3 * H * H, tm->p, (size_t)2 * H * H * 2, cudaMemcpyDeviceToDevice));
    *hb += (int64_t)2 * H * H * 2;
    drop(c, h + ".final_layer.adaLN_modulation.1.weight");
    const int NS = std::max(d.max_diffusion_steps, 1);
    RET(dmalloc(c, &c->temb, (size_t)NS * H));
    RET(dmalloc(c, &c->coef_dev, (size_t)NS));
    RET(dmalloc(c, &c->tfreqs, 128));
    std::vector<float> fr(128);
    for (int j = 0; j < 128; ++j) fr[j] = expf((-9.210340371976184f * (float)j) / 128.0f);
    CK(cudaMemcpy(c->tfreqs, fr.data(), 128 * 4, cudaMemcpyHostToDevice));
    RET(dmalloc(c, &c->s_tfeat, (size_t)NS * 256));
    RET(dmalloc(c, &c->s_t1, (size_t)NS * H));
    RET(dmalloc(c, &c->s_condp, (size_t)M2 * H));
    RET(dmalloc(c, &c->s_call, (size_t)NS * M2 * H));
    RET(dmalloc(c, &c->s_mod, (size_t)NS * M2 * modrows));
    RET(dmalloc(c, &c->cfg_dev, 4));
    RET(dmalloc(c, &c->gridbar, 2));
    RET(dmalloc(c, &c->st_bar, 32));
    if (getenv("VV_STREAM_TRACE")) {
      c->st_trace_cta = atoi(getenv("VV_STREAM_TRACE"));
      c->st_trace_ops = 4096;
      RET(dmalloc(c, &c->st_trace, (size_t)c->st_trace_ops * ST_TRACE));
      RET(dmalloc(c, &c->st_trace2, (size_t)c->st_trace_ops * c->sm_count * 2));
    }
    CK(cudaHostAlloc((void**)&c->st_diag_host, 64, cudaHostAllocMapped));
    memset(c->st_diag_host, 0, 64);
    CK(cudaHostGetDevicePointer((void**)&c->st_diag_dev, c->st_diag_host, 0));
    RET(dmalloc(c, &c->s_hx, (size_t)M2 * H));
    RET(dmalloc(c, &c->s_hg, (size_t)M2 * F));
    RET(dmalloc(c, &c->s_hgu, (size_t)2 * M2 * 2 * F));
    RET(dmalloc(c, &c->s_v, (size_t)M2 * 64));
    RET(dmalloc(c, &c->s_z, (size_t)2 * B * 64));
    RET(dmalloc(c, &c->s_x0, (size_t)2 * B * 64));
  }
  {
    int64_t* cb = &c->wbytes[5];
    const std::string a = "model.acoustic_connector", s = "model.semantic_connector";
    RET(take_bf16(c, a + ".fc1.weight", {H, d.acoustic_vae_dim}, &c->ca_fc1, cb));
    RET(take_f32(c, a + ".fc1.bias", {H}, &c->ca_b1, cb));
    RET(take_f32(c, a + ".norm.weight", {H}, &c->ca_n, cb));
    RET(take_bf16(c, a + ".fc2.weight", {H, H}, &c->ca_fc2, cb));
    RET(take_f32(c, a + ".fc2.bias", {H}, &c->ca_b2, cb));
    RET(take_bf16(c, s + ".fc1.weight", {H, d.semantic_vae_dim}, &c->cs_fc1, cb));
    RET(take_f32(c, s + ".fc1.bias", {H}, &c->cs_b1, cb));
    RET(take_f32(c, s + ".norm.weight", {H}, &c->cs_n, cb));
    RET(take_bf16(c, s + ".fc2.weight", {H, H}, &c->cs_fc2, cb));
    RET(take_f32(c, s + ".fc2.bias", {H}, &c->cs_b2, cb));
    RET(dmalloc(c, &c->s_e, (size_t)B * H));
    RET(dmalloc(c, &c->s_c1, (size_t)B * H));
    RET(dmalloc(c, &c->s_feat, (size_t)B * d.semantic_vae_dim));
    RET(dmalloc(c, &c->s_audio, (size_t)B * 3200 * 4));
    RET(dmalloc(c, &c->s_latent, (size_t)B * 64));
  }
  int hop = 1;
  for (int i = 0; i < d.n_stages - 1; ++i) hop *= d.dec_ratios[i];
  size_t max_tc = 0, max_win = 0;
  {
    Codec& k = c->dec;
    int64_t* kb = &c->wbytes[3];
    std::vector<StateSeg> segs;
    const std::string p = "model.acoustic_tokenizer.decoder";
    const int ns = d.n_stages, nf = d.dec_n_filters;
    k.convs.resize(ns + 1); k.stages.resize(ns); k.T.resize(ns); k.C.resize(ns);
    int T = 1;
    for (int i = 0; i < ns; ++i) {
      const int C = nf << (ns - 1 - i);
      if (i == 0) RET(build_conv(c, p + ".upsample_layers.0.0.conv.conv", d.acoustic_vae_dim, C, 7, 1, &k.convs[0], kb, &segs));
      else { RET(build_convtr(c, S("%s.upsample_layers.%d.0.convtr.convtr", p.c_str(), i), C * 2, C, d.dec_ratios[i - 1], &k.convs[i], kb, &segs)); T *= d.dec_ratios[i - 1]; }
      k.T[i] = T; k.C[i] = C;
      max_tc = std::max(max_tc, (size_t)T * C);
      max_win = std::max(max_win, (size_t)(T + 8) * C * 2);
      k.stages[i].resize(d.dec_depths[i]);
      for (int j = 0; j < d.dec_depths[i]; ++j) RET(build_block(c, S("%s.stages.%d.%d", p.c_str(), i, j), C, &k.stages[i][j], kb, &segs));
    }
    RET(build_conv(c, p + ".head.conv.conv", nf, 1, 7, 1, &k.convs[ns], kb, &segs));
    if (T != hop) return fail(VV_ERR_INVALID, "decoder hop mismatch");
    RET(upload_segs(c, &k, segs));
    k.weight_bytes = *kb;
  }
  {
    Codec& k = c->enc;
    int64_t* kb = &c->wbytes[4];
    std::vector<StateSeg> segs;
    const std::string p = "model.semantic_tokenizer.encoder";
    const int ns = d.n_stages, nf = d.enc_n_filters;
    k.convs.resize(ns + 1); k.stages.resize(ns); k.T.resize(ns); k.C.resize(ns);
    int T = hop;
    for (int i = 0; i < ns; ++i) {
      const int C = nf << i;
      if (i == 0) RET(build_conv(c, p + ".downsample_layers.0.0.conv.conv", 1, C, 7, 1, &k.convs[0], kb, &segs));
      else {
        const int r = d.enc_ratios[ns - 1 - i];
        RET(build_conv(c, S("%s.downsample_layers.%d.0.conv.conv", p.c_str(), i), C / 2, C, 2 * r, r, &k.convs[i], kb, &segs));
        if (T % r) return fail(VV_ERR_INVALID, "encoder ratio mismatch");
        T /= r;
      }
      k.T[i] = T; k.C[i] = C;
      max_tc = std::max(max_tc, (size_t)T * C);
      max_win = std::max(max_win, (size_t)(T + 16) * C * 2);
      k.stages[i].resize(d.enc_depths[i]);
      for (int j = 0; j < d.enc_depths[i]; ++j) RET(build_block(c, S("%s.stages.%d.%d", p.c_str(), i, j), C, &k.stages[i][j], kb, &segs));
    }
    if (T != 1) return fail(VV_ERR_INVALID, "encoder hop mismatch");
    RET(build_conv(c, p + ".head.conv.conv", nf << (ns - 1), d.semantic_vae_dim, 7, 1, &k.convs[ns], kb, &segs));
    RET(upload_segs(c, &k, segs));
    k.weight_bytes = *kb;
  }
  max_win = std::max(max_win, (size_t)(hop + 8) * 64);
  RET(dmalloc(c, &c->s_xa, (size_t)B * max_tc));
  RET(dmalloc(c, &c->s_xb, (size_t)B * max_tc));
  RET(dmalloc(c, &c->s_xn, (size_t)B * max_tc));
  RET(dmalloc(c, &c->s_u, (size_t)B * max_tc * 4));
  RET(dmalloc(c, &c->s_win, (size_t)B * max_win));
  c->planes_elems = std::max<size_t>((size_t)B * max_tc * 4, (size_t)std::max(d.max_diffusion_steps, 1) * M2 * H);
  RET(dmalloc(c, &c->s_planes, 2 * c->planes_elems));
  RET(dmalloc(c, &c->s_h, (size_t)M2 * H));
  RET(dmalloc(c, &c->s_qkv, (size_t)M2 * c->Nqkv));
  RET(dmalloc(c, &c->s_qrot, (size_t)M2 * nq));
  RET(dmalloc(c, &c->s_attn, (size_t)M2 * nq));
  RET(dmalloc(c, &c->s_act, (size_t)M2 * I));
  RET(dmalloc(c, &c->s_lgu, (size_t)M2 * 2 * I));
  RET(dmalloc(c, &c->s_rope, (size_t)M2 * HD));
  RET(dmalloc(c, &c->s_cx, (size_t)2 * B * 8192));
  RET(dmalloc(c, &c->s_cu, (size_t)2 * B * 32768));
  RET(dmalloc(c, &c->s_pacc2, (size_t)M2 * d.num_kv_heads * c->sm_count * 8 * HD));
  RET(dmalloc(c, &c->s_pml2, (size_t)M2 * d.num_kv_heads * c->sm_count * 8 * 2));
  RET(dmalloc(c, &c->s_pacc, (size_t)M2 * d.num_q_heads * c->nsplit * HD));
  RET(dmalloc(c, &c->s_pml, (size_t)M2 * d.num_q_heads * c->nsplit * 2));
  RET(dmalloc(c, &c->s_tok, 64));
  RET(dmalloc(c, &c->kv_len_dev, 16));
  RET(dmalloc(c, &c->row_mode_dev, 16));
  {
    int ones[16];
    for (int i = 0; i < 16; ++i) ones[i] = 1;
    CK(cudaMemcpy(c->row_mode_dev, ones, sizeof ones, cudaMemcpyHostToDevice));
  }
  c->kv_len_host.assign(M2, 0);
  c->seq_pages.assign(M2, {});
  for (auto& r : c->raw) if (r.second.p) { cudaFree(r.second.p); r.second.p = nullptr; }
  CK(cudaDeviceSynchronize());
  c->finalized = true;
  return 0;
}

extern "C" int64_t vv_weight_bytes(vv_ctx* c, int which) { return (c && which >= 0 && which < 6) ? c->wbytes[which] : -1; }
extern "C" int64_t vv_launch_count(vv_ctx* c) { return c ? c->launches : -1; }

template <class F>
static int run_cached(vv_ctx* c, const std::string& key, cudaStream_t s, F&& enqueue) {
  if (!c->use_graphs || s == nullptr) { L l{c, s}; return enqueue(l); }
  auto it = c->graphs.find(key);
  if (it == c->graphs.end()) {
    const int64_t before = c->launches;
    CK(cudaStreamBeginCapture(s, cudaStreamCaptureModeThreadLocal));
    L l{c, s};
    int r = enqueue(l);
    cudaGraph_t g = nullptr;
    cudaError_t e = cudaStreamEndCapture(s, &g);
    if (r < 0) { if (g) cudaGraphDestroy(g); return r; }
    if (e != cudaSuccess) return fail(VV_ERR_CUDA, "graph capture failed (%s): %s", key.c_str(), cudaGetErrorString(e));
    GraphEntry ge;
    ge.launches = c->launches - before;
    c->launches = before;
    e = cudaGraphInstantiate(&ge.exec, g, 0);
    cudaGraphDestroy(g);
    if (e != cudaSuccess) return fail(VV_ERR_CUDA, "graph instantiate failed: %s", cudaGetErrorString(e));
    it = c->graphs.emplace(key, ge).first;
  }
  CK(cudaGraphLaunch(it->second.exec, s));
  c->launches += it->second.launches;
  return 0;
}

template <class T>
static void dfree(vv_ctx* c, T** p) {
  if (!*p) return;
  auto it = std::find(c->allocs.begin(), c->allocs.end(), (void*)*p);
  if (it != c->allocs.end()) c->allocs.erase(it);
  cudaFree(*p);
  *p = nullptr;
}
static void drop_graphs(vv_ctx* c, std::initializer_list<const char*> prefixes) {
  for (auto it = c->graphs.begin(); it != c->graphs.end();) {
    bool hit = false;
    for (const char* pre : prefixes) hit = hit || it->first.rfind(pre, 0) == 0;
    if (hit) { cudaGraphExecDestroy(it->second.exec); it = c->graphs.erase(it); }
    else ++it;
  }
}

extern "C" int vv_kv_init(vv_ctx* c, int64_t n_pages) {
  if (!c || !c->finalized) return fail(VV_ERR_STATE, "vv_kv_init before vv_finalize_weights");
  if (n_pages < 2 * c->d.max_batch) return fail(VV_ERR_INVALID, "vv_kv_init: need at least one page per sequence (%d)", 2 * c->d.max_batch);
  CK(cudaSetDevice(c->device));
  if (c->kpool) {
    CK(cudaDeviceSynchronize());
    dfree(c, &c->kpool); dfree(c, &c->vpool); dfree(c, &c->page_table_dev);
    drop_graphs(c, {"lm:", "lmr:", "frame:"});
    for (auto it = c->sprogs.begin(); it != c->sprogs.end();) {
      if (it->first.rfind("lmf:", 0) == 0) { dfree(c, &it->second.ops); dfree(c, &it->second.tmaps); it = c->sprogs.erase(it); }
      else ++it;
    }
    std::fill(c->kv_len_host.begin(), c->kv_len_host.end(), 0);
    for (auto& pg : c->seq_pages) pg.clear();
  }
  const auto& d = c->d;
  const size_t per_layer = (size_t)n_pages * d.num_kv_heads * KV_PAGE * d.head_dim;
  RET(dmalloc(c, &c->kpool, per_layer * d.num_layers));
  RET(dmalloc(c, &c->vpool, per_layer * d.num_layers));
  c->n_pages = n_pages;
  c->max_pages = (int)n_pages;
  const size_t nt = (size_t)2 * d.max_batch * c->max_pages;
  RET(dmalloc(c, &c->page_table_dev, nt));
  c->free_pages.clear();
  for (int i = (int)n_pages - 1; i >= 0; --i) c->free_pages.push_back(i);
  return 0;
}
extern "C" int64_t vv_kv_pages_free(vv_ctx* c) { return c ? (int64_t)c->free_pages.size() : -1; }
extern "C" int64_t vv_kv_pages_total(vv_ctx* c) { return c ? c->n_pages : -1; }
extern "C" int64_t vv_kv_len(vv_ctx* c, int seq) { return (c && seq >= 0 && seq < (int)c->kv_len_host.size()) ? c->kv_len_host[seq] : -1; }

struct PageVals { int v[32]; };
__global__ void page_table_set_kernel(int* dst, PageVals pv, int n) { if ((int)threadIdx.x < n) dst[threadIdx.x] = pv.v[threadIdx.x]; }

extern "C" int vv_kv_reserve(vv_ctx* c, int seq, int64_t n_tokens, void* stream) {
  if (!c || !c->kpool) return fail(VV_ERR_STATE, "KV pool not initialised");
  if (seq < 0 || seq >= 2 * c->d.max_batch) return fail(VV_ERR_INVALID, "bad seq %d", seq);
  auto& pg = c->seq_pages[seq];
  const int64_t needp = (n_tokens + KV_PAGE - 1) / KV_PAGE;
  if (needp > c->max_pages) return fail(VV_ERR_NOMEM, "KV page pool too small (seq %d needs %lld pages of %d)", seq, (long long)needp, c->max_pages);
  size_t first = pg.size();
  while ((int64_t)pg.size() < needp) {
    if (c->free_pages.empty()) return fail(VV_ERR_NOMEM, "KV page pool exhausted (seq %d needs %lld pages)", seq, (long long)needp);
    pg.push_back(c->free_pages.back());
    c->free_pages.pop_back();
  }
  while (first < pg.size()) {
    PageVals pv;
    const int n = (int)std::min<size_t>(32, pg.size() - first);
    for (int i = 0; i < 32; ++i) pv.v[i] = i < n ? pg[first + i] : 0;
    page_table_set_kernel<<<1, 32, 0, (cudaStream_t)stream>>>(c->page_table_dev + (size_t)seq * c->max_pages + first, pv, n);
    CKL();
    c->launches++;
    first += n;
  }
  return 0;
}
static void release_pages(vv_ctx* c, int seq, int64_t len) {
  auto& pg = c->seq_pages[seq];
  const size_t keep = (size_t)((len + KV_PAGE - 1) / KV_PAGE);
  while (pg.size() > keep) { c->free_pages.push_back(pg.back()); pg.pop_back(); }
}

struct Lens { int v[16]; };
__global__ void kv_set_all_kernel(int* kv_len, Lens l, int n) { if (threadIdx.x < n) kv_len[threadIdx.x] = l.v[threadIdx.x]; }

static int push_lens(vv_ctx* c, cudaStream_t s) {
  Lens l;
  const int n = 2 * c->d.max_batch;
  for (int i = 0; i < 16; ++i) l.v[i] = i < n ? (int)c->kv_len_host[i] : 0;
  kv_set_all_kernel<<<1, 32, 0, s>>>(c->kv_len_dev, l, n);
  CKL();
  c->launches++;
  return 0;
}
// ... 310 lines not shown
  CK(cudaStreamSynchronize(s));
  L l{c, s};
  GemvP p = mk(c->h_t0, nullptr, c->s_tfeat, 256, c->s_t1, H, n_steps, H, 256);
  p.epi = EPI_SILU;
  RET(linear(l, p));
  p = mk(c->h_t2, nullptr, c->s_t1, H, c->temb, H, n_steps, H, H);
  RET(linear(l, p));
  CK(cudaStreamSynchronize(s));
  c->n_steps = n_steps;
  drop_graphs(c, {"tail:", "diff:", "frame:"});
  return 0;
}

static void head_step_gemvs(vv_ctx* c, int i, std::vector<GemvP>* out) {
  const auto& d = c->d;
  const int H = d.hidden_size, F = d.head_ffn_dim, M = 2 * d.max_batch, LH = d.head_layers;
  const int modld = (3 * LH + 2) * H;
  const float* mod = c->s_mod + (size_t)i * M * modld;
  for (int li = 0; li < LH; ++li) {
    const HeadLayer& hl = c->head[li];
    GemvP p = mk(hl.wgu, nullptr, c->s_hx, H, c->s_hg, F, M, 2 * F, H);
    p.pro = PRO_ADALN; p.pro_w = hl.norm; p.pro_eps = d.head_rms_eps;
    p.pro_shift = mod + (size_t)li * 3 * H; p.pro_scale = mod + (size_t)li * 3 * H + H; p.pro_ld = modld;
    p.epi = EPI_SWIGLU;
    out->push_back(p);
    p = mk(hl.wdown, nullptr, c->s_hg, F, c->s_hx, H, M, H, F);
    p.epi = EPI_GATED_RESID; p.epi_a = mod + (size_t)li * 3 * H + 2 * H; p.epi_lda = modld; p.res = c->s_hx; p.ldres = H;
    out->push_back(p);
  }
  GemvP p = mk(c->h_final, nullptr, c->s_hx, H, c->s_v, 64, M, 64, H);
  p.pro = PRO_ADALN; p.pro_w = nullptr; p.pro_eps = d.head_rms_eps;
  p.pro_shift = mod + (size_t)LH * 3 * H; p.pro_scale = mod + (size_t)LH * 3 * H + H; p.pro_ld = modld;
  out->push_back(p);
}
__global__ void set_float_kernel(float* p, float v) { *p = v; }
static int set_cfg(vv_ctx* c, float cfg, cudaStream_t s) {
  if (memcmp(&cfg, &c->cfg_last, sizeof(float)) == 0) return 0;
  set_float_kernel<<<1, 1, 0, s>>>(c->cfg_dev, cfg);
  CKL();
  c->launches++;
  c->cfg_last = cfg;
  return 0;
}

static int sampler_stream_prog(vv_ctx* c, const float* noise, float* latent_out, const vv_ctx::StreamProg** out) {
  char key[256];
  snprintf(key, sizeof key, "samp:%p:%p:%d:%d:%p:%d", (const void*)noise, (void*)latent_out, c->n_steps, (int)c->sde, (const void*)c->step_noise,
           c->coef_version);
  auto it = c->sprogs.find(key);
  if (it != c->sprogs.end()) { *out = &it->second; return 0; }
  const auto& d = c->d;
  const int H = d.hidden_size, F = d.head_ffn_dim, B = d.max_batch, M = 2 * B, LH = d.head_layers, N = c->n_steps;
  const long long modld = (long long)(3 * LH + 2) * H;
  StreamBuilder b(c);
  auto dpm = [&](int i) {
    SDpm o;
    memset(&o, 0, sizeof o);
    if (i < 0) { o.z_in = c->s_z + B * 64; o.z_out = c->s_z; o.x0_in = c->s_x0 + B * 64; o.x0_out = c->s_x0; }
    else {
      o.z_in = c->s_z + (size_t)(i & 1) * B * 64; o.z_out = c->s_z + (size_t)((i + 1) & 1) * B * 64;
      o.x0_in = c->s_x0 + (size_t)(i & 1) * B * 64; o.x0_out = c->s_x0 + (size_t)((i + 1) & 1) * B * 64;
    }
    o.v = c->s_v; o.noise = noise; o.cfg_p = c->cfg_dev; o.step_noise = c->sde ? c->step_noise : nullptr;
    o.latent_out = (i == N - 1) ? latent_out : nullptr; o.step = i; o.B = B;
    if (i >= 0) o.c = c->coef_host[i];
    return o;
  };
  auto proj = [&](int i, bool sync) -> int {
    SOp* o;
    RET(b.gemv(c->h_noisy, nullptr, nullptr, 0, c->s_hx, H, M, H, 64, sync, &o));
    o->pro = SP_DPM; o->store = 1; o->dpm = dpm(i);
    return 0;
  };
  float* gu[2] = {c->s_hgu, c->s_hgu + (size_t)M * 2 * F};
  RET(proj(-1, false));
  b.ops.back().init_dst = gu[0]; b.ops.back().init_n = (long long)M * 2 * F;
  for (int i = 0; i < N; ++i) {
    const float* mod = c->s_mod + (size_t)i * M * modld;
    for (int li = 0; li < LH; ++li) {
      const HeadLayer& hl = c->head[li];
      SOp* o;
      RET(b.gemv(hl.wgu, nullptr, c->s_hx, H, gu[li & 1], 2 * F, M, 2 * F, H, true, &o));
      o->pro = SP_ADALN; o->pro_w = hl.norm; o->pro_eps = d.head_rms_eps;
      o->pro_shift = mod + (size_t)li * 3 * H; o->pro_scale = mod + (size_t)li * 3 * H + H; o->pro_ld = modld;
      o->init_dst = gu[(li + 1) & 1]; o->init_n = (long long)M * 2 * F;
      RET(b.gemv(hl.wdown, nullptr, gu[li & 1], 2 * F, c->s_hx, H, M, H, F, true, &o));
      o->pro = SP_SWIGLU; o->alpha_kind = SA_GATE; o->alpha = mod + (size_t)li * 3 * H + 2 * H; o->lda = modld;
      if (li == 0) { o->init_dst = c->s_v; o->init_n = (long long)M * 64; }
    }
    SOp* o;
    RET(b.gemv(c->h_final, nullptr, c->s_hx, H, c->s_v, 64, M, 64, H, true, &o));
    o->pro = SP_ADALN; o->pro_w = nullptr; o->pro_eps = d.head_rms_eps;
    o->pro_shift = mod + (size_t)LH * 3 * H; o->pro_scale = mod + (size_t)LH * 3 * H + H; o->pro_ld = modld;
    RET(proj(i, true));
  }
  vv_ctx::StreamProg pr;
  RET(finish_stream(b, &pr));
  it = c->sprogs.emplace(key, pr).first;
  *out = &it->second;
  return 0;
}

static int enqueue_diffusion(const L& l, const float* cond, const float* noise, float* latent_out, const vv_ctx::StreamProg* sprog) {
  vv_ctx* c = l.c;
  const auto& d = c->d;
  const int H = d.hidden_size, B = d.max_batch, M = 2 * B, LH = d.head_layers, N = c->n_steps;
  if (N < 1) return fail(VV_ERR_STATE, "vv_set_diffusion_steps not called");
  const int modld = (3 * LH + 2) * H;
  if (c->sde && !c->step_noise) return fail(VV_ERR_STATE, "sde-dpmsolver++ needs vv_set_step_noise before sampling");
  GemvP p = mk(c->h_cond, nullptr, cond, H, c->s_condp, H, M, H, H);
  RET(linear(l, p));
  {
    const long long n = (long long)N * M * H;
    CK(launch_k(l, head_cond_prep_kernel, dim3((unsigned)((n + 255) / 256)), dim3(256), 0, c->s_condp, c->temb, c->s_call, N, M, H));
  }
  p = mk(c->h_mod, nullptr, c->s_call, H, c->s_mod, modld, N * M, modld, H);
  RET(linear(l, p));
  if (sprog) return launch_stream(l, *sprog);
  CK(launch_k(l, dpm_update_proj_kernel, dim3(B, (H + 255) / 256), dim3(256), 0, c->s_z + B * 64, c->s_z, c->s_x0 + B * 64, c->s_x0, c->s_v, noise,
              c->coef_dev, -1, (const float*)c->cfg_dev, c->h_noisy, c->s_hx, nullptr, B, H, 1, (const float*)nullptr));
  L lh = l;
  if (c->l2_persist_bytes && c->head_slab_bytes) {
    lh.win_base = c->head_slab;
    lh.win_bytes = std::min(c->head_slab_bytes, c->l2_window_max);
    lh.win_ratio = std::min(1.0f, (float)c->l2_persist_bytes / (float)lh.win_bytes);
  }
  for (int i = 0; i < N; ++i) {
    std::vector<GemvP> g;
    head_step_gemvs(c, i, &g);
    for (auto& q : g) RET(linear(lh, q));
    const bool last = (i == N - 1);
    const float* z_in = c->s_z + (size_t)(i & 1) * B * 64; float* z_out = c->s_z + (size_t)((i + 1) & 1) * B * 64;
    const float* x0_in = c->s_x0 + (size_t)(i & 1) * B * 64; float* x0_out = c->s_x0 + (size_t)((i + 1) & 1) * B * 64;
    CK(launch_k(l, dpm_update_proj_kernel, dim3(B, last ? 1 : (H + 255) / 256), dim3(256), 0, z_in, z_out, x0_in, x0_out, (const float*)c->s_v, noise,
                (const DpmCoef*)c->coef_dev, i, (const float*)c->cfg_dev, (const bf16*)c->h_noisy, c->s_hx, last ? latent_out : (float*)nullptr, B, H,
                last ? 0 : 1, c->sde ? c->step_noise : (const float*)nullptr));
  }
  return 0;
}

extern "C" int vv_diffusion_sample(vv_ctx* c, const float* cond, const float* noise, const int32_t* active, float cfg, float* latent_out,
                                   void* stream) {
  (void)active;
  if (!c || !c->finalized) return fail(VV_ERR_STATE, "not finalized");
  CK(cudaSetDevice(c->device));
  RET(set_cfg(c, cfg, (cudaStream_t)stream));
  char key[256];
  snprintf(key, sizeof key, "diff:%p:%p:%p", (const void*)cond, (const void*)noise, (void*)latent_out);
  const vv_ctx::StreamProg* sprog = nullptr;
  if (c->use_stream & 1) RET(sampler_stream_prog(c, noise, latent_out, &sprog));
  return run_cached(c, key, (cudaStream_t)stream, [&](const L& l) { return enqueue_diffusion(l, cond, noise, latent_out, sprog); });
}

static int assemble(const L& l, const float* src, const float* hist, float* win, float* next, int B, int T, int ctx, int C,
                    const float* norm_w, float eps, float alpha, float beta) {
  const int rows = B * (ctx + T);
  if (C >= 512) CK(launch_k(l, assemble_window_block_kernel, dim3(rows), dim3(256), 0, src, hist, win, next, B, T, ctx, C, norm_w, eps, alpha, beta));
  else CK(launch_k(l, assemble_window_kernel, dim3((rows + 7) / 8), dim3(256), 0, src, hist, win, next, B, T, ctx, C, norm_w, eps, alpha, beta));
  return 0;
}

static int enqueue_block(const L& l, const Block& b, const float* xin, float* xout, int B, int T, float eps) {
  vv_ctx* c = l.c;
  const int C = b.C, M = B * T;
  RET(assemble(l, xin, b.hist, c->s_win, b.next, B, T, 6, C, b.norm_w, eps, 1.f, 0.f));
  {
    const long long n = (long long)M * C;
    CK(launch_k(l, dwconv_res_kernel, dim3((unsigned)((n + 255) / 256)), dim3(256), 0, xin, c->s_win, b.dw_w, b.dw_b, b.gamma, xout, B, T, C));
  }
  GemvP p;
  if (M < c->mma_min_rows || (c->ring_rms && c->mma_ring && C <= MR_MAXK_NORM && c->use_wgmma != 2)) {
    p = mk(b.w1, b.b1, xout, C, c->s_u, 4 * C, M, 4 * C, C);
    p.pro = PRO_RMSNORM; p.pro_w = b.ffn_norm_w; p.pro_eps = eps; p.epi = EPI_GELU;
    RET(linear(l, p));
  } else {
    if (C >= 512) CK(launch_k(l, rows_norm_block_kernel, dim3(M), dim3(256), 0, xout, b.ffn_norm_w, c->s_xn, C, eps));
    else CK(launch_k(l, rows_norm_kernel, dim3((M + 7) / 8), dim3(256), 0, xout, b.ffn_norm_w, c->s_xn, M, C, eps));
    p = mk(b.w1, b.b1, c->s_xn, C, c->s_u, 4 * C, M, 4 * C, C);
    p.epi = EPI_GELU;
    RET(linear(l, p));
  }
  p = mk(b.w2, b.b2, c->s_u, 4 * C, xout, C, M, C, 4 * C);
  p.epi = EPI_GAMMA_RESID; p.epi_a = b.ffn_gamma; p.res = xout; p.ldres = C;
  return linear(l, p);
}

static int conv_apply(const L& l, const ConvL& cv, const float* win, float* y, int B, int T_out, int T_in) {
  RowMap xm; xm.T = T_out; xm.bs = (long long)(cv.ctx + T_in) * cv.Cin; xm.rs = (long long)cv.stride * cv.Cin;
  const int M = B * T_out;
  if (cv.wf) {
    const long long n = (long long)M * cv.N;
    if (cv.K >= 64) CK(launch_k(l, conv_warp_kernel, dim3((unsigned)((n + 7) / 8)), dim3(256), 0, cv.wf, cv.bias, win, xm, y, M, cv.N, cv.K));
    else CK(launch_k(l, conv_naive_kernel, dim3((unsigned)((n + 255) / 256)), dim3(256), 0, cv.wf, cv.bias, win, xm, y, M, cv.N, cv.K));
    return 0;
  }
  GemvP p = mk(cv.w, cv.bias, win, 0, y, cv.N, M, cv.N, cv.K);
  p.xmap = xm;
  return linear(l, p);
}

struct ScopedMinRows {
  vv_ctx* c; int saved;
  ScopedMinRows(vv_ctx* c_, int v) : c(c_), saved(c_->mma_min_rows) { c->mma_min_rows = v; }
  ~ScopedMinRows() { c->mma_min_rows = saved; }
};

static bool codec_stream_stage(const vv_ctx* c, const Codec& k, int i) {
  const long long rows = (long long)c->d.max_batch * k.T[i];
  return (c->use_stream & 8) && k.T[i] <= 8 && rows <= 32;
}
static long long codec_x_floats(const vv_ctx* c) { return (long long)c->d.max_batch * 8192; }
static long long codec_u_floats(const vv_ctx* c) { return (long long)c->d.max_batch * 32768; }
static void window_op(SOp* o, const ConvL& cv, const float* src, int T_in, int T_out, int row_stride, float alpha, float beta) {
  o->pro = SP_WINDOW;
  SCodec& w = o->cod;
  memset(&w, 0, sizeof w);
  w.hist = cv.hist; w.next = cv.next; w.src = src; w.ctx = cv.ctx; w.T_in = T_in; w.T_out = T_out; w.stride = row_stride; w.cin = cv.Cin;
  w.alpha = alpha; w.beta = beta;
}
struct CodecBufs {
  float* X[2]; float* U[2];
  int cur = 0, ub = 0;
  explicit CodecBufs(vv_ctx* c) { X[0] = c->s_cx; X[1] = c->s_cx + codec_x_floats(c); U[0] = c->s_cu; U[1] = c->s_cu + codec_u_floats(c); }
};
static int stage_ops(StreamBuilder& b, vv_ctx* c, CodecBufs& cb, const std::vector<Block>& blocks, int B, int T, bool zero_for_next, float* extra_zero,
                     long long extra_n) {
  for (size_t j = 0; j < blocks.size(); ++j) {
    const Block& blk = blocks[j];
    const int C = blk.C, M = B * T;
    SOp* o;
    {
      SOp& mx = b.push(SK_MIX, true);
      mx.M = M; mx.K = C; mx.x = cb.X[cb.cur]; mx.ldx = C;
      SCodec& w = mx.cod;
      memset(&w, 0, sizeof w);
      w.hist = blk.hist; w.next = blk.next; w.T_out = T; w.norm_w = blk.norm_w; w.dw_w = blk.dw_w; w.dw_b = blk.dw_b; w.gamma = blk.gamma;
      w.x1_out = cb.X[cb.cur ^ 1]; w.eps = c->d.codec_eps;
    }
    RET(b.gemv(blk.w1, blk.b1, cb.X[cb.cur ^ 1], C, cb.U[cb.ub], 4 * C, M, 4 * C, C, true, &o));
    o->pro = SP_RMSNORM; o->pro_w = blk.ffn_norm_w; o->pro_eps = c->d.codec_eps;
    o->init_dst = cb.U[cb.ub ^ 1]; o->init_n = codec_u_floats(c);
    RET(b.gemv(blk.w2, blk.b2, cb.U[cb.ub], 4 * C, cb.X[cb.cur ^ 1], C, M, C, 4 * C, true, &o));
    o->pro = SP_GELU; o->alpha_kind = SA_GAMMA; o->alpha = blk.ffn_gamma;
    if (j + 1 == blocks.size()) {
      if (zero_for_next) { o->init_dst = cb.X[cb.cur]; o->init_n = codec_x_floats(c); }
      if (extra_zero) { o->init2_dst = extra_zero; o->init2_n = extra_n; }
    }
    cb.cur ^= 1; cb.ub ^= 1;
  }
  return 0;
}

static int dec_front_prog(vv_ctx* c, const float* latent, const vv_ctx::StreamProg** out, int* n_front, float** out_x) {
  Codec& k = c->dec;
  const auto& d = c->d;
  const int B = d.max_batch;
  int nf = 0;
  while (nf < d.n_stages - 1 && codec_stream_stage(c, k, nf)) ++nf;
  *n_front = nf; *out = nullptr; *out_x = nullptr;
  if (nf == 0) return 0;
  char key[96];
  snprintf(key, sizeof key, "decf:%p", (const void*)latent);
  {
    auto hit = c->sprogs.find(key);
    if (hit != c->sprogs.end()) { *out = &hit->second; *out_x = c->dec_front_x; return 0; }
  }
  CodecBufs cb(c);
  StreamBuilder b(c);
  b.nop(false, cb.X[0], codec_x_floats(c));
  b.ops.back().init2_dst = cb.U[0]; b.ops.back().init2_n = codec_u_floats(c);
  SOp* o;
  RET(b.gemv(k.convs[0].w, k.convs[0].bias, nullptr, 0, cb.X[0], k.convs[0].N, B, k.convs[0].N, k.convs[0].K, true, &o));
  window_op(o, k.convs[0], latent, 1, 1, 1, 1.0f / c->speech_scale, -c->speech_bias);
  for (int i = 0; i < nf; ++i) {
    if (i > 0) {
      const ConvL& cv = k.convs[i];
      const int Tin = k.T[i - 1];
      RET(b.gemv(cv.w, cv.bias, nullptr, 0, cb.X[cb.cur ^ 1], cv.N, B * Tin, cv.N, cv.K, true, &o));
      window_op(o, cv, cb.X[cb.cur], Tin, Tin, 1, 1.f, 0.f);
      cb.cur ^= 1;
    }
    RET(stage_ops(b, c, cb, k.stages[i], B, k.T[i], i + 1 < nf, nullptr, 0));
  }
  *out_x = c->dec_front_x = cb.X[cb.cur];
  auto it = c->sprogs.find(key);
  if (it == c->sprogs.end()) {
    vv_ctx::StreamProg pr;
    RET(finish_stream(b, &pr));
    it = c->sprogs.emplace(key, pr).first;
  }
  *out = &it->second;
  return 0;
}

static int enc_back_first(const vv_ctx* c) {
  const Codec& k = c->enc;
  int f = c->d.n_stages;
  while (f > 1 && codec_stream_stage(c, k, f - 1)) --f;
  return f;
}
static int enc_back_prog(vv_ctx* c, const float* xin, float* feat, const vv_ctx::StreamProg** out) {
  Codec& k = c->enc;
  const auto& d = c->d;
  const int B = d.max_batch, ns = d.n_stages, f = enc_back_first(c);
  *out = nullptr;
  if (f >= ns) return 0;
  char key[96];
  snprintf(key, sizeof key, "encb:%p:%p", (const void*)xin, (void*)feat);
  auto it = c->sprogs.find(key);
  if (it != c->sprogs.end()) { *out = &it->second; return 0; }
  CodecBufs cb(c);
  StreamBuilder b(c);
  b.nop(false, cb.X[0], codec_x_floats(c));
  b.ops.back().init2_dst = cb.U[0]; b.ops.back().init2_n = codec_u_floats(c);
  SOp* o;
  for (int i = f; i < ns; ++i) {
    const ConvL& cv = k.convs[i];
    const int Tin = k.T[i - 1], Tout = k.T[i];
    float* dst = (i == f) ? cb.X[0] : cb.X[cb.cur ^ 1];
    RET(b.gemv(cv.w, cv.bias, nullptr, 0, dst, cv.N, B * Tout, cv.N, cv.K, true, &o));
    window_op(o, cv, i == f ? xin : cb.X[cb.cur], Tin, Tout, cv.stride, 1.f, 0.f);
    if (i > f) cb.cur ^= 1;
    const bool last = (i + 1 == ns);
    RET(stage_ops(b, c, cb, k.stages[i], B, Tout, !last, last ? feat : nullptr, (long long)B * d.semantic_vae_dim));
  }
  const ConvL& hd = k.convs[ns];
  RET(b.gemv(hd.w, hd.bias, nullptr, 0, feat, hd.N, B, hd.N, hd.K, true, &o));
  window_op(o, hd, cb.X[cb.cur], 1, 1, 1, 1.f, 0.f);
  vv_ctx::StreamProg pr;
  RET(finish_stream(b, &pr));
  it = c->sprogs.emplace(key, pr).first;
  *out = &it->second;
  return 0;
}

static int enqueue_decode(const L& l, const float* latent, const int32_t* active, float* audio, const vv_ctx::StreamProg* front = nullptr,
                          int n_front = 0, float* front_x = nullptr) {
  vv_ctx* c = l.c;
  ScopedMinRows scoped(c, c->codec_mma_min_rows);
  const auto& d = c->d;
  Codec& k = c->dec;
  const int B = d.max_batch, ns = d.n_stages;
  float *xa = c->s_xa, *xb = c->s_xb;
  if (front) {
    RET(launch_stream(l, *front));
    xa = front_x;
  } else {
    n_front = 0;
    RET(assemble(l, latent, k.convs[0].hist, c->s_win, k.convs[0].next, B, 1, 6, 64, nullptr, 0.f, 1.0f / c->speech_scale, -c->speech_bias));
    RET(conv_apply(l, k.convs[0], c->s_win, xa, B, 1, 1));
  }
  for (int i = n_front; i < ns; ++i) {
    if (i > 0) {
      const ConvL& cv = k.convs[i];
      const int Tin = k.T[i - 1];
      RET(assemble(l, xa, cv.hist, c->s_win, cv.next, B, Tin, 1, cv.Cin, nullptr, 0.f, 1.f, 0.f));
      RowMap xm; xm.T = Tin; xm.bs = (long long)(1 + Tin) * cv.Cin; xm.rs = cv.Cin;
      float* dst = (xa == c->s_xa) ? c->s_xb : c->s_xa;
      GemvP p = mk(cv.w, cv.bias, c->s_win, 0, dst, cv.N, B * Tin, cv.N, cv.K);
      p.xmap = xm;
      RET(linear(l, p));
      xa = dst; xb = (xa == c->s_xa) ? c->s_xb : c->s_xa;
    }
    for (const Block& b : k.stages[i]) { RET(enqueue_block(l, b, xa, xb, B, k.T[i], d.codec_eps)); std::swap(xa, xb); }
  }
  const ConvL& hd = k.convs[ns];
  const int T = k.T[ns - 1];
  RET(assemble(l, xa, hd.hist, c->s_win, hd.next, B, T, 6, hd.Cin, nullptr, 0.f, 1.f, 0.f));
  RET(conv_apply(l, hd, c->s_win, audio, B, T, T));
  CK(launch_k(l, advance_kernel, dim3(k.n_segs, B, ADV_SLICES), dim3(256), 0, k.segs_dev, active));
  return 0;
}

static float* encode_front_out(vv_ctx* c, int first) {
  const Codec& k = c->enc;
  bool in_a = true;
  for (int i = 0; i < first; ++i) {
    if (i > 0) in_a = !in_a;
    if (k.stages[i].size() & 1) in_a = !in_a;
  }
  return in_a ? c->s_xa : c->s_xb;
}
static int enqueue_encode(const L& l, const float* audio, const int32_t* active, float* feat, const vv_ctx::StreamProg* back = nullptr) {
  vv_ctx* c = l.c;
  ScopedMinRows scoped(c, c->codec_mma_min_rows);
  const auto& d = c->d;
  Codec& k = c->enc;
  const int B = d.max_batch, ns = d.n_stages;
  const int stop = back ? enc_back_first(c) : ns;
  float *xa = c->s_xa, *xb = c->s_xb;
  int hop = k.T[0];
  RET(assemble(l, audio, k.convs[0].hist, c->s_win, k.convs[0].next, B, hop, 6, 1, nullptr, 0.f, 1.f, 0.f));
  RET(conv_apply(l, k.convs[0], c->s_win, xa, B, hop, hop));
  for (int i = 0; i < stop; ++i) {
    if (i > 0) {
      const ConvL& cv = k.convs[i];
      const int Tin = k.T[i - 1];
      RET(assemble(l, xa, cv.hist, c->s_win, cv.next, B, Tin, cv.ctx, cv.Cin, nullptr, 0.f, 1.f, 0.f));
      RET(conv_apply(l, cv, c->s_win, xb, B, k.T[i], Tin));
      std::swap(xa, xb);
    }
    for (const Block& b : k.stages[i]) { RET(enqueue_block(l, b, xa, xb, B, k.T[i], d.codec_eps)); std::swap(xa, xb); }
  }
  if (back) {
    if (xa != encode_front_out(c, stop)) return fail(VV_ERR_STATE, "encoder hand-off buffer mismatch");
    RET(launch_stream(l, *back));
  } else {
    const ConvL& hd = k.convs[ns];
    RET(assemble(l, xa, hd.hist, c->s_win, hd.next, B, 1, 6, hd.Cin, nullptr, 0.f, 1.f, 0.f));
    RET(conv_apply(l, hd, c->s_win, feat, B, 1, 1));
  }
  CK(launch_k(l, advance_kernel, dim3(k.n_segs, B, ADV_SLICES), dim3(256), 0, k.segs_dev, active));
  return 0;
}

static int enqueue_connect(const L& l, const float* latent, const float* sem, const int32_t* active, float* embeds) {
  vv_ctx* c = l.c;
  const auto& d = c->d;
  const int H = d.hidden_size, B = d.max_batch;
  GemvP p = mk(c->ca_fc1, c->ca_b1, latent, 64, c->s_c1, H, B, H, 64);
  RET(linear(l, p));
  p = mk(c->ca_fc2, c->ca_b2, c->s_c1, H, c->s_e, H, B, H, H);
  p.pro = PRO_RMSNORM; p.pro_w = c->ca_n; p.pro_eps = 1e-6f;
  RET(linear(l, p));
  p = mk(c->cs_fc1, c->cs_b1, sem, d.semantic_vae_dim, c->s_c1, H, B, H, d.semantic_vae_dim);
  RET(linear(l, p));
  p = mk(c->cs_fc2, c->cs_b2, c->s_c1, H, c->s_e, H, B, H, H);
  p.pro = PRO_RMSNORM; p.pro_w = c->cs_n; p.pro_eps = 1e-6f; p.epi = EPI_RESID; p.res = c->s_e; p.ldres = H;
  RET(linear(l, p));
  CK(launch_k(l, select_embeds_kernel, dim3(B), dim3(256), 0, embeds, c->s_e, active, B, H));
  return 0;
}

extern "C" int vv_codec_decode_frame(vv_ctx* c, const float* latent, const int32_t* active, float* audio_out, void* stream) {
  if (!c || !c->finalized) return fail(VV_ERR_STATE, "not finalized");
  CK(cudaSetDevice(c->device));
  char key[256];
  snprintf(key, sizeof key, "dec:%p:%p:%p", (const void*)latent, (const void*)active, (void*)audio_out);
  const vv_ctx::StreamProg* front = nullptr; int nf = 0; float* fx = nullptr;
  RET(dec_front_prog(c, latent, &front, &nf, &fx));
  return run_cached(c, key, (cudaStream_t)stream, [&](const L& l) { return enqueue_decode(l, latent, active, audio_out, front, nf, fx); });
}
extern "C" int vv_semantic_encode_frame(vv_ctx* c, const float* audio, const int32_t* active, float* feat_out, void* stream) {
  if (!c || !c->finalized) return fail(VV_ERR_STATE, "not finalized");
  CK(cudaSetDevice(c->device));
  char key[256];
  snprintf(key, sizeof key, "enc:%p:%p:%p", (const void*)audio, (const void*)active, (void*)feat_out);
  const vv_ctx::StreamProg* back = nullptr;
  RET(enc_back_prog(c, encode_front_out(c, enc_back_first(c)), feat_out, &back));
  return run_cached(c, key, (cudaStream_t)stream, [&](const L& l) { return enqueue_encode(l, audio, active, feat_out, back); });
}
extern "C" int vv_connect(vv_ctx* c, const float* latent, const float* sem, const int32_t* active, float* embeds, void* stream) {
  if (!c || !c->finalized) return fail(VV_ERR_STATE, "not finalized");
  CK(cudaSetDevice(c->device));
  L l{c, (cudaStream_t)stream};
  return enqueue_connect(l, latent, sem, active, embeds);
}
extern "C" int vv_frame_tail(vv_ctx* c, const float* hidden, const float* noise, const int32_t* active, float cfg, float* latent_out,
                             float* audio_out, float* embeds, void* stream) {
  if (!c || !c->finalized) return fail(VV_ERR_STATE, "not finalized");
  CK(cudaSetDevice(c->device));
  char key[320];
  RET(set_cfg(c, cfg, (cudaStream_t)stream));
  snprintf(key, sizeof key, "tail:%p:%p:%p:%p:%p:%p", (const void*)hidden, (const void*)noise, (const void*)active, (void*)latent_out,
           (void*)audio_out, (void*)embeds);
  const vv_ctx::StreamProg* sprog = nullptr;
  if (c->use_stream & 1) RET(sampler_stream_prog(c, noise, latent_out, &sprog));
  const vv_ctx::StreamProg *front = nullptr, *back = nullptr; int nf = 0; float* fx = nullptr;
  RET(dec_front_prog(c, latent_out, &front, &nf, &fx));
  RET(enc_back_prog(c, encode_front_out(c, enc_back_first(c)), c->s_feat, &back));
  return run_cached(c, key, (cudaStream_t)stream, [&](const L& l) {
    RET(enqueue_diffusion(l, hidden, noise, latent_out, sprog));
    RET(enqueue_decode(l, latent_out, active, audio_out, front, nf, fx));
    RET(enqueue_encode(l, audio_out, active, c->s_feat, back));
    return enqueue_connect(l, latent_out, c->s_feat, active, embeds);
  });
}

struct Rows { int v[16]; };
__global__ void state_zero_val_kernel(const StateSeg* __restrict__ segs, Rows r) {
  const int b = r.v[blockIdx.y];
  const StateSeg s = segs[blockIdx.x];
  float* dd = s.hist + (size_t)b * s.n;
  for (int i = threadIdx.x; i < s.n; i += blockDim.x) dd[i] = 0.f;
}
extern "C" int vv_codec_state_zero(vv_ctx* c, const int32_t* rows_host, int n, void* stream) {
  if (!c || !c->finalized) return fail(VV_ERR_STATE, "not finalized");
  if (n < 1) return 0;
  if (n > c->d.max_batch) return fail(VV_ERR_INVALID, "too many rows");
  Rows r;
  for (int i = 0; i < 16; ++i) r.v[i] = i < n ? rows_host[i] : 0;
  for (int i = 0; i < n; ++i) if (r.v[i] < 0 || r.v[i] >= c->d.max_batch) return fail(VV_ERR_INVALID, "row %d out of range", r.v[i]);
  cudaStream_t s = (cudaStream_t)stream;
  state_zero_val_kernel<<<dim3(c->dec.n_segs, n), 256, 0, s>>>(c->dec.segs_dev, r);
  CKL();
  state_zero_val_kernel<<<dim3(c->enc.n_segs, n), 256, 0, s>>>(c->enc.segs_dev, r);
  CKL();
  c->launches += 2;
  return 0;
}
extern "C" int vv_codec_state_reset(vv_ctx* c, void* stream) {
  if (!c || !c->finalized) return fail(VV_ERR_STATE, "not finalized");
  int rows[8];
  for (int i = 0; i < c->d.max_batch; ++i) rows[i] = i;
  return vv_codec_state_zero(c, rows, c->d.max_batch, stream);
}

extern "C" int vv_debug_gemv(vv_ctx* c, const void* w, const float* bias, const float* x, float* y, int M, int N, int K, int prologue,
                             const float* pro_w, float eps, int epilogue, void* stream) {
  if (!c) return fail(VV_ERR_INVALID, "null ctx");
  CK(cudaSetDevice(c->device));
  L l{c, (cudaStream_t)stream};
  const int ldy = epilogue == EPI_SWIGLU ? N / 2 : N;
  GemvP p = mk((const bf16*)w, bias, x, K, y, ldy, M, N, K);
  p.pro = prologue; p.pro_w = pro_w; p.pro_eps = eps; p.epi = epilogue;
  if (epilogue == EPI_RESID) { p.res = y; p.ldres = N; }
  return linear(l, p);
}

static int run_debug_stream(vv_ctx* c, StreamBuilder& b, void* stream) {
  vv_ctx::StreamProg pr;
  int rc = finish_stream(b, &pr);
  if (rc == 0) {
    L l{c, (cudaStream_t)stream};
    rc = launch_stream(l, pr);
    if (rc == 0 && cudaStreamSynchronize((cudaStream_t)stream) != cudaSuccess) rc = fail(VV_ERR_CUDA, "stream kernel: %s", cudaGetErrorString(cudaGetLastError()));
  }
  if (pr.ops) dfree(c, &pr.ops);
  if (pr.tmaps) dfree(c, &pr.tmaps);
  for (bf16* t : b.owned) dfree(c, &t);
  if (rc < 0) return rc;
  if (c->st_diag_host[0]) return fail(VV_ERR_CUDA, "stream kernel watchdog: code %u cta %u thread %u a %u b %u c %u", c->st_diag_host[0], c->st_diag_host[1],
                                      c->st_diag_host[2], c->st_diag_host[3], c->st_diag_host[4], c->st_diag_host[5]);
  return pr.n_ops;
}

extern "C" int vv_debug_stream_gemv(vv_ctx* c, const void* w, const float* bias, const float* x, float* y, int M, int N, int K, int pro,
                                    const float* pro_w, float eps, int alpha_kind, const float* alpha, int accumulate, void* stream) {
  if (!c || !c->finalized) return fail(VV_ERR_STATE, "not finalized");
  CK(cudaSetDevice(c->device));
  StreamBuilder b(c);
  b.fresh_weights = true;
  if (!accumulate) b.nop(false, y, (long long)M * N);
  SOp* o;
  RET(b.gemv((const bf16*)w, bias, x, pro == SP_SWIGLU ? 2LL * K : (long long)K, y, N, M, N, K, !accumulate, &o));
  o->pro = pro; o->pro_w = pro_w; o->pro_eps = eps; o->alpha_kind = alpha_kind; o->alpha = alpha; o->lda = N;
  const int rc = run_debug_stream(c, b, stream);
  return rc < 0 ? rc : 0;
}

extern "C" int vv_debug_stream_gemv2(vv_ctx* c, const void* w, const float* bias, const float* x, int64_t ldx, float* y, int64_t ldy, int M, int N, int K,
                                     int pro, const float* pro_w, float eps, const float* pro_shift, const float* pro_scale, int64_t pro_ld,
                                     int alpha_kind, const float* alpha, int64_t lda, int store, int64_t operand_cap, void* stream) {
  if (!c || !c->finalized) return fail(VV_ERR_STATE, "not finalized");
  if (pro != SP_NONE && pro != SP_RMSNORM && pro != SP_ADALN && pro != SP_SWIGLU && pro != SP_GELU && pro != SP_SILU)
    return fail(VV_ERR_INVALID, "vv_debug_stream_gemv2: prologue %d not supported", pro);
  if (alpha_kind != SA_ONE && alpha_kind != SA_GATE && alpha_kind != SA_GAMMA) return fail(VV_ERR_INVALID, "vv_debug_stream_gemv2: alpha_kind %d", alpha_kind);
  if ((pro == SP_ADALN && (!pro_shift || !pro_scale)) || (alpha_kind != SA_ONE && !alpha))
    return fail(VV_ERR_INVALID, "vv_debug_stream_gemv2: missing AdaLN / alpha operand");
  if (ldx < (pro == SP_SWIGLU ? 2LL * K : (long long)K) || ldy < N || (alpha_kind == SA_GATE && lda < N) || (pro == SP_ADALN && pro_ld < K) ||
      ((uintptr_t)x & 15) || ldx % 4 || (pro == SP_ADALN && (pro_ld % 4 || ((uintptr_t)pro_shift & 15) || ((uintptr_t)pro_scale & 15))))
    return fail(VV_ERR_INVALID, "vv_debug_stream_gemv2: strides must cover the row and keep rows 16-byte aligned");
  CK(cudaSetDevice(c->device));
  StreamBuilder b(c);
  b.fresh_weights = true;
  b.operand_cap = operand_cap;
  SOp* o;
  RET(b.gemv((const bf16*)w, bias, x, ldx, y, ldy, M, N, K, false, &o));
  o->pro = pro; o->pro_w = pro_w; o->pro_eps = eps; o->pro_shift = pro_shift; o->pro_scale = pro_scale; o->pro_ld = pro_ld;
  o->alpha_kind = alpha_kind; o->alpha = alpha; o->lda = lda; o->store = store ? 1 : 0;
  return run_debug_stream(c, b, stream);
}
extern "C" int vv_stream_trace_read2(vv_ctx* c, long long* out, int max_ops) {
  if (!c || !c->st_trace2) return 0;
  CK(cudaDeviceSynchronize());
  const int n = std::min(max_ops, c->st_trace_last_ops);
  CK(cudaMemcpy(out, c->st_trace2, (size_t)n * c->sm_count * 2 * sizeof(long long), cudaMemcpyDeviceToHost));
  return c->sm_count;
}
extern "C" int vv_stream_trace_read(vv_ctx* c, long long* out, int* out_meta, int max_ops, const char* prog_prefix) {
  if (!c || !c->st_trace) return 0;
  CK(cudaDeviceSynchronize());
  const int n = std::min(max_ops, c->st_trace_last_ops);
  CK(cudaMemcpy(out, c->st_trace, (size_t)n * ST_TRACE * sizeof(long long), cudaMemcpyDeviceToHost));
  for (auto& kv : c->sprogs) {
    if (kv.first.rfind(prog_prefix, 0) != 0 || kv.second.n_ops != c->st_trace_last_ops) continue;
    std::vector<SOp> ops(kv.second.n_ops);
    CK(cudaMemcpy(ops.data(), kv.second.ops, ops.size() * sizeof(SOp), cudaMemcpyDeviceToHost));
    for (int i = 0; i < n; ++i) { out_meta[4 * i] = ops[i].kind; out_meta[4 * i + 1] = ops[i].N; out_meta[4 * i + 2] = ops[i].K; out_meta[4 * i + 3] = ops[i].pro; }
    break;
  }
  return n;
}
extern "C" int vv_stream_diag(vv_ctx* c, unsigned* out6) {
  if (!c || !c->st_diag_host) return fail(VV_ERR_STATE, "no context");
  for (int i = 0; i < 6; ++i) out6[i] = c->st_diag_host[i];
  return 0;
}

extern "C" int vv_debug_barrier_bench(vv_ctx* c, int iters, int per_sm, float* ms_out) {
  if (!c || !c->finalized) return fail(VV_ERR_STATE, "not finalized");
  CK(cudaSetDevice(c->device));
  cudaStream_t s;
  CK(cudaStreamCreate(&s));
  cudaLaunchConfig_t cfg;
  memset(&cfg, 0, sizeof cfg);
  cfg.gridDim = dim3(c->sm_count * per_sm); cfg.blockDim = dim3(256); cfg.stream = s;
  cudaLaunchAttribute attr[1];
  attr[0].id = cudaLaunchAttributeCooperative; attr[0].val.cooperative = 1;
  cfg.attrs = attr; cfg.numAttrs = 1;
  float* sink = c->s_v;
  cudaEvent_t e0, e1;
  CK(cudaEventCreate(&e0)); CK(cudaEventCreate(&e1));
  CK(cudaLaunchKernelEx(&cfg, barrier_bench_kernel, c->gridbar, 10, sink));
  CK(cudaEventRecord(e0, s));
  CK(cudaLaunchKernelEx(&cfg, barrier_bench_kernel, c->gridbar, iters, sink));
  CK(cudaEventRecord(e1, s));
  CK(cudaStreamSynchronize(s));
  CK(cudaEventElapsedTime(ms_out, e0, e1));
  cudaEventDestroy(e0); cudaEventDestroy(e1); cudaStreamDestroy(s);
  return 0;
}
```

Baseline: 22.71.

## Fuse codec ConvNeXt block into single tensor-core kernel with split-bf16 MMA

Replaces the multi-kernel codec block sequence (window assembly with RMSNorm, depthwise conv plus residual, FFN linear layers) with one fused kernel. The fused kernel stages weights through cp.async, computes the norm and depthwise conv in shared memory, and runs both FFN matmuls on mma.sync using hi/lo bf16 splitting of the activations to keep near-fp32 accuracy. When the hidden dimension is split across CTAs it accumulates with atomics into buffers that earlier kernels zero, and it rotates buffers through a TailRot helper. The aim is to cut launch count and intermediate global memory traffic in the codec decode and encode paths, at the cost of extra MMA work from the split precision and atomic contention.

```diff
diff --git a/include/vibevoice_b200.h b/include/vibevoice_b200.h
--- a/include/vibevoice_b200.h
+++ b/include/vibevoice_b200.h
@@ -97,6 +97,9 @@
 int vv_debug_stream_gemv2(vv_ctx* ctx, const void* w_bf16, const float* bias, const float* x, int64_t ldx, float* y, int64_t ldy, int M, int N,
                           int K, int prologue, const float* pro_w, float eps, const float* pro_shift, const float* pro_scale, int64_t pro_ld,
                           int alpha_kind, const float* alpha, int64_t lda, int store, int64_t operand_cap, void* stream);
+int vv_debug_codec_block(vv_ctx* ctx, int B, int T, int C, const float* norm_w, const float* dw_w, const float* dw_b, const float* gamma,
+                         const float* ffn_norm_w, const void* w1_bf16, const float* b1, const void* w2_bf16, const float* b2, const float* ffn_gamma,
+                         const float* x, const float* hist, float* next, float* out, void* stream);
 int vv_stream_trace_read2(vv_ctx* ctx, long long* out , int max_ops);
 int vv_stream_trace_read(vv_ctx* ctx, long long* out , int* out_meta , int max_ops, const char* program_prefix);
 int vv_stream_diag(vv_ctx* ctx, unsigned* out6);
diff --git a/vibevoice_b200/_native.py b/vibevoice_b200/_native.py
--- a/vibevoice_b200/_native.py
+++ b/vibevoice_b200/_native.py
@@ -74,6 +74,7 @@
     "vv_debug_gemv": (_I, [_P, _P, _P, _P, _P, _I, _I, _I, _I, _P, _F, _I, _P]),
     "vv_debug_stream_gemv": (_I, [_P, _P, _P, _P, _P, _I, _I, _I, _I, _P, _F, _I, _P, _I, _P]),
     "vv_debug_stream_gemv2": (_I, [_P, _P, _P, _P, _L, _P, _L, _I, _I, _I, _I, _P, _F, _P, _P, _L, _I, _P, _L, _I, _L, _P]),
+    "vv_debug_codec_block": (_I, [_P, _I, _I, _I] + [_P] * 15),
     "vv_stream_diag": (_I, [_P, _P]),
     "vv_stream_trace_read": (_I, [_P, _P, _P, _I, C.c_char_p]),
     "vv_stream_trace_read2": (_I, [_P, _P, _I]),
diff --git a/vibevoice_b200/csrc/vv_kernels.cuh b/vibevoice_b200/csrc/vv_kernels.cuh
--- a/vibevoice_b200/csrc/vv_kernels.cuh
+++ b/vibevoice_b200/csrc/vv_kernels.cuh
@@ -41,6 +41,7 @@
   const float* res;
   int ldres;
   int WK;
+  int y_zeroed;
 };
 
 VV_DEVINL void pdl_trigger() { asm volatile("griddepcontrol.launch_dependents;" ::: "memory"); }
@@ -768,9 +769,10 @@
 
 __global__ void assemble_window_kernel(const float* __restrict__ src, const float* __restrict__ hist,
                                        float* __restrict__ win, float* __restrict__ hist_next, int B, int T, int ctx, int C,
-                                       const float* __restrict__ norm_w, float eps, float alpha, float beta) {
-  pdl_trigger();
-  pdl_wait();
+                                       float alpha, float beta, float* __restrict__ zero_dst, long long zero_n) {
+  pdl_trigger();
+  pdl_wait();
+  for (long long i = (long long)blockIdx.x * blockDim.x + threadIdx.x; i < zero_n; i += (long long)gridDim.x * blockDim.x) zero_dst[i] = 0.f;
   const int row = blockIdx.x * (blockDim.x >> 5) + (threadIdx.x >> 5);
   const int lane = threadIdx.x & 31;
   const int R = ctx + T;
@@ -783,15 +785,8 @@
     for (int c = lane; c < C; c += 32) { float v = hr[c]; wr[c] = v; if (hn) hn[c] = v; }
   } else {
     const float* sr = src + ((size_t)b * T + (j - ctx)) * C;
-    float inv = 1.f;
-    if (norm_w) {
-      float ss = 0.f;
-      for (int c = lane; c < C; c += 32) { float v = sr[c]; ss += v * v; }
-      ss = warp_sum(ss);
-      inv = rsqrtf(ss / (float)C + eps);
-    }
     for (int c = lane; c < C; c += 32) {
-      float v = norm_w ? sr[c] * inv * norm_w[c] : sr[c] * alpha + beta;
+      const float v = sr[c] * alpha + beta;
       wr[c] = v;
       if (hn) hn[c] = v;
     }
@@ -800,35 +795,23 @@
 
 __global__ void __launch_bounds__(256) assemble_window_block_kernel(const float* __restrict__ src, const float* __restrict__ hist,
                                                                     float* __restrict__ win, float* __restrict__ hist_next, int B, int T,
-                                                                    int ctx, int C, const float* __restrict__ norm_w, float eps, float alpha,
-                                                                    float beta) {
-  pdl_trigger();
-  pdl_wait();
+                                                                    int ctx, int C, float alpha, float beta, float* __restrict__ zero_dst,
+                                                                    long long zero_n) {
+  pdl_trigger();
+  pdl_wait();
+  for (long long i = (long long)blockIdx.x * blockDim.x + threadIdx.x; i < zero_n; i += (long long)gridDim.x * blockDim.x) zero_dst[i] = 0.f;
   const int row = blockIdx.x, tid = threadIdx.x;
   const int R = ctx + T;
   const int b = row / R, j = row % R;
   float* wr = win + ((size_t)b * R + j) * C;
   float* hn = (j >= T) ? hist_next + ((size_t)b * ctx + (j - T)) * C : nullptr;
-  __shared__ float sp[8];
   if (j < ctx) {
     const float* hr = hist + ((size_t)b * ctx + j) * C;
     for (int c = tid; c < C; c += 256) { float v = hr[c]; wr[c] = v; if (hn) hn[c] = v; }
   } else {
     const float* sr = src + ((size_t)b * T + (j - ctx)) * C;
-    float inv = 1.f;
-    if (norm_w) {
-      float ss = 0.f;
-      for (int c = tid; c < C; c += 256) { float v = sr[c]; ss += v * v; }
-      ss = warp_sum(ss);
-      if ((tid & 31) == 0) sp[tid >> 5] = ss;
-      __syncthreads();
-      float t = 0.f;
-#pragma unroll
-      for (int i = 0; i < 8; ++i) t += sp[i];
-      inv = rsqrtf(t / (float)C + eps);
-    }
     for (int c = tid; c < C; c += 256) {
-      float v = norm_w ? sr[c] * inv * norm_w[c] : sr[c] * alpha + beta;
+      const float v = sr[c] * alpha + beta;
       wr[c] = v;
       if (hn) hn[c] = v;
     }
@@ -853,21 +836,230 @@
   for (int c = tid; c < C; c += 256) y[(size_t)row * C + c] = xr[c] * inv * (w ? w[c] : 1.f);
 }
 
-__global__ void dwconv_res_kernel(const float* __restrict__ x, const float* __restrict__ win, const float* __restrict__ w ,
-                                  const float* __restrict__ bias, const float* __restrict__ gamma, float* __restrict__ out,
-                                  int B, int T, int C) {
-  pdl_trigger();
-  pdl_wait();
-  const long long idx = (long long)blockIdx.x * blockDim.x + threadIdx.x;
-  if (idx >= (long long)B * T * C) return;
-  const int c = (int)(idx % C);
-  const long long bt = idx / C;
-  const int t = (int)(bt % T), b = (int)(bt / T);
-  const float* wp = win + ((size_t)b * (T + 6) + t) * C + c;
-  float acc = bias[c];
-#pragma unroll
-  for (int j = 0; j < 7; ++j) acc = fmaf(w[j * C + c], wp[(size_t)j * C], acc);
-  out[idx] = x[idx] + gamma[c] * acc;
+constexpr int CB_R = 16, CB_HC = 64, CB_KT = 64, CB_NCOL = 512, CB_NST = 3;
+struct CodecBlockP {
+  const float* x; float* out; const float* hist; float* next;
+  const float *norm_w, *dw_w , *dw_b, *gamma, *ffn_norm_w, *b1, *b2, *ffn_gamma;
+  const bf16 *w1 , *w2 ;
+  float* zero_dst; long long zero_n;
+  int T, C, tiles, spc, ncol;
+  float eps;
+};
+struct CodecBlockSmem {
+  int rv, kp, a_ld, w2, x1, w1, pr, u, h, a, total;
+  VV_DEVINL __host__ CodecBlockSmem(int C, int T, int ncol, int spc) {
+    rv = T < CB_R ? T : CB_R;
+    kp = C < 16 ? 16 : C;
+    a_ld = kp + 8;
+    w2 = 0;
+    x1 = w2 + ncol * (CB_HC + 8) * 2;
+    w1 = x1 + rv * C * 4;
+    pr = w1 + CB_NST * CB_HC * ((kp < CB_KT ? kp : CB_KT) + 8) * 2;
+    u = pr + (11 * C + CB_HC * spc + 2 * ncol) * 4;
+    h = u;
+    a = h + 2 * CB_R * (CB_HC + 8) * 2;
+    const int a_end = a + 2 * (rv + 1) * a_ld * 2, win_end = u + (rv + 6) * C * 4;
+    total = a_end > win_end ? a_end : win_end;
+  }
+};
+VV_DEVINL void ldmatrix_x2(unsigned (&r)[2], const void* smem) {
+  unsigned sa = (unsigned)__cvta_generic_to_shared(smem);
+  asm volatile("ldmatrix.sync.aligned.m8n8.x2.shared.b16 {%0,%1}, [%2];" : "=r"(r[0]), "=r"(r[1]) : "r"(sa));
+}
+VV_DEVINL void split_store_bf16x2(bf16* hi, bf16* lo, float a, float b) {
+  const float ha = __bfloat162float(__float2bfloat16_rn(a)), hb = __bfloat162float(__float2bfloat16_rn(b));
+  *reinterpret_cast<unsigned*>(hi) = pack_bf16(ha, hb);
+  *reinterpret_cast<unsigned*>(lo) = pack_bf16(a - ha, b - hb);
+}
+
+__global__ void __launch_bounds__(256) codec_block_kernel(CodecBlockP p) {
+  extern __shared__ __align__(16) unsigned char cb_smem[];
+  const int tid = threadIdx.x, lane = tid & 31, warp = tid >> 5;
+  const int C = p.C, T = p.T, H4 = 4 * C;
+  const CodecBlockSmem L(C, T, p.ncol, p.spc);
+  const int b = blockIdx.x / p.tiles, t0 = (blockIdx.x % p.tiles) * CB_R;
+  const int rows = min(CB_R, T - t0);
+  const int chunk = blockIdx.y, col0 = blockIdx.z * p.ncol;
+  const int kt_w = L.kp < CB_KT ? L.kp : CB_KT, kt_ld = kt_w + 8, nkt = (L.kp + CB_KT - 1) / CB_KT;
+  bf16* sW2 = reinterpret_cast<bf16*>(cb_smem + L.w2);
+  float* sX1 = reinterpret_cast<float*>(cb_smem + L.x1);
+  bf16* sW1 = reinterpret_cast<bf16*>(cb_smem + L.w1);
+  float* sWin = reinterpret_cast<float*>(cb_smem + L.u);
+  bf16* sHh = reinterpret_cast<bf16*>(cb_smem + L.h);
+  bf16* sHl = sHh + CB_R * (CB_HC + 8);
+  bf16* sAh = reinterpret_cast<bf16*>(cb_smem + L.a);
+  bf16* sAl = sAh + (L.rv + 1) * L.a_ld;
+  float* sNw = reinterpret_cast<float*>(cb_smem + L.pr);
+  float *sDw = sNw + C, *sDb = sDw + 7 * C, *sGm = sDb + C, *sFn = sGm + C, *sB1 = sFn + C, *sB2 = sB1 + CB_HC * p.spc, *sFg = sB2 + p.ncol;
+
+  auto load_w1 = [&](int sub, int kt) {
+    bf16* dst = sW1 + (kt % CB_NST) * CB_HC * kt_ld;
+    const int cpr = kt_w / 8;
+    for (int i = tid; i < CB_HC * cpr; i += 256) {
+      const int r = i / cpr, cc = (i % cpr) * 8, n = sub * CB_HC + r, k = kt * CB_KT + cc;
+      const bool ok = n < H4 && k < C;
+      cp_async16(dst + r * kt_ld + cc, p.w1 + (ok ? (size_t)n * C + k : 0), ok ? 16 : 0);
+    }
+  };
+  auto load_w2 = [&](int sub) {
+    for (int i = tid; i < p.ncol * 8; i += 256) {
+      const int r = i >> 3, cc = (i & 7) * 8, h = sub * CB_HC + cc;
+      const bool ok = h < H4;
+      cp_async16(sW2 + r * (CB_HC + 8) + cc, p.w2 + (ok ? (size_t)(col0 + r) * H4 + h : 0), ok ? 16 : 0);
+    }
+  };
+  auto issue_sub = [&](int sub) {
+    load_w2(sub); load_w1(sub, 0); cp_async_commit();
+    if (nkt > 1) load_w1(sub, 1);
+    cp_async_commit();
+  };
+  const int sub0 = chunk * p.spc;
+
+  pdl_trigger();
+  {
+    auto stage = [&](float* dst, const float* src, int n, int valid) {
+      for (int i = tid * 4; i < n; i += 1024) cp_async16(dst + i, src + (i < valid ? i : 0), i < valid ? 16 : 0);
+    };
+    stage(sNw, p.norm_w, C, C); stage(sDw, p.dw_w, 7 * C, 7 * C); stage(sDb, p.dw_b, C, C); stage(sGm, p.gamma, C, C);
+    stage(sFn, p.ffn_norm_w, C, C); stage(sB1, p.b1 + sub0 * CB_HC, CB_HC * p.spc, H4 - sub0 * CB_HC);
+    stage(sB2, p.b2 + col0, p.ncol, p.ncol); stage(sFg, p.ffn_gamma + col0, p.ncol, p.ncol);
+  }
+  issue_sub(sub0);
+  pdl_wait();
+  if (p.zero_dst)
+    for (long long i = ((long long)(blockIdx.z * gridDim.y + blockIdx.y) * gridDim.x + blockIdx.x) * 256 + tid; i < p.zero_n;
+         i += (long long)gridDim.x * gridDim.y * gridDim.z * 256)
+      p.zero_dst[i] = 0.f;
+
+  const float* xb = p.x + (size_t)b * T * C;
+  {
+    const int c4 = C / 4, nw = (rows + 6) * c4;
+    for (int i = tid; i < nw + rows * c4; i += 256) {
+      if (i < nw) {
+        const int j = i / c4, c = (i % c4) * 4, t = t0 - 6 + j;
+        cp_async16(sWin + j * C + c, t < 0 ? p.hist + ((size_t)b * 6 + (t + 6)) * C + c : xb + (size_t)t * C + c, 16);
+      } else {
+        const int r = (i - nw) / c4, c = ((i - nw) % c4) * 4;
+        cp_async16(sX1 + r * C + c, xb + (size_t)(t0 + r) * C + c, 16);
+      }
+    }
+    cp_async_commit();
+    cp_async_wait<0>();
+    __syncthreads();
+  }
+  const bool write_next = chunk == 0 && blockIdx.z == 0 && t0 + rows == T;
+  for (int j = warp; j < rows + 6; j += 8) {
+    const int t = t0 - 6 + j;
+    float* wr = sWin + j * C;
+    if (t >= 0) {
+      float ss = 0.f;
+      for (int c = lane * 4; c < C; c += 128) {
+        const float4 v = *reinterpret_cast<const float4*>(wr + c);
+        ss += v.x * v.x + v.y * v.y + v.z * v.z + v.w * v.w;
+      }
+      const float inv = rsqrtf(warp_sum(ss) / (float)C + p.eps);
+      for (int c = lane * 4; c < C; c += 128) {
+        const float4 v = *reinterpret_cast<const float4*>(wr + c), w = *reinterpret_cast<const float4*>(sNw + c);
+        *reinterpret_cast<float4*>(wr + c) = make_float4(v.x * inv * w.x, v.y * inv * w.y, v.z * inv * w.z, v.w * inv * w.w);
+      }
+    }
+    if (write_next && t >= T - 6) {
+      float* nr = p.next + ((size_t)b * 6 + (t - (T - 6))) * C;
+      for (int c = lane * 4; c < C; c += 128) *reinterpret_cast<float4*>(nr + c) = *reinterpret_cast<const float4*>(wr + c);
+    }
+  }
+  __syncthreads();
+  for (int i = tid; i < rows * C; i += 256) {
+    const int r = i / C, c = i % C;
+    float acc = sDb[c];
+#pragma unroll
+    for (int j = 0; j < 7; ++j) acc = fmaf(sDw[j * C + c], sWin[(r + j) * C + c], acc);
+    sX1[i] += sGm[c] * acc;
+  }
+  __syncthreads();
+  for (int r = warp; r <= L.rv; r += 8) {
+    bf16 *ah = sAh + r * L.a_ld, *al = sAl + r * L.a_ld;
+    float inv = 0.f;
+    if (r < rows) {
+      float ss = 0.f;
+      for (int c = lane; c < C; c += 32) { const float v = sX1[r * C + c]; ss += v * v; }
+      inv = rsqrtf(warp_sum(ss) / (float)C + p.eps);
+    }
+    for (int c = lane * 2; c < L.kp; c += 64) {
+      float v0 = 0.f, v1 = 0.f;
+      if (r < rows && c < C) { v0 = sX1[r * C + c] * inv * sFn[c]; v1 = sX1[r * C + c + 1] * inv * sFn[c + 1]; }
+      split_store_bf16x2(ah + c, al + c, v0, v1);
+    }
+  }
+
+  const int ntile = p.ncol / 8, tpw = (ntile + 7) / 8, nt0 = warp * tpw;
+  float oacc[8][4];
+#pragma unroll
+  for (int i = 0; i < 8; ++i)
+#pragma unroll
+    for (int q = 0; q < 4; ++q) oacc[i][q] = 0.f;
+  const int arow = (lane & 15) < rows ? (lane & 15) : L.rv;
+  const int g = lane >> 2, q2 = (lane & 3) * 2;
+  for (int s = 0; s < p.spc; ++s) {
+    const int sub = sub0 + s;
+    if (s > 0) issue_sub(sub);
+    float hacc[4] = {0.f, 0.f, 0.f, 0.f};
+    for (int kt = 0; kt < nkt; ++kt) {
+      cp_async_wait<1>();
+      __syncthreads();
+      if (kt + 2 < nkt) load_w1(sub, kt + 2);
+      cp_async_commit();
+      const bf16* wt = sW1 + (kt % CB_NST) * CB_HC * kt_ld;
+      for (int kk = 0; kk < kt_w; kk += 16) {
+        const int k = kt * CB_KT + kk;
+        unsigned ah[4], al[4], bw[2];
+        ldmatrix_x4(ah, sAh + arow * L.a_ld + k + (lane >> 4) * 8);
+        ldmatrix_x4(al, sAl + arow * L.a_ld + k + (lane >> 4) * 8);
+        ldmatrix_x2(bw, wt + (warp * 8 + (lane & 7)) * kt_ld + kk + ((lane >> 3) & 1) * 8);
+        mma_bf16_16816(hacc, ah, bw[0], bw[1]);
+        mma_bf16_16816(hacc, al, bw[0], bw[1]);
+      }
+    }
+    {
+      const int hc = warp * 8 + q2;
+      const float bb0 = sB1[s * CB_HC + hc], bb1 = sB1[s * CB_HC + hc + 1];
+      split_store_bf16x2(sHh + g * (CB_HC + 8) + hc, sHl + g * (CB_HC + 8) + hc, gelu_erf_f(hacc[0] + bb0), gelu_erf_f(hacc[1] + bb1));
+      split_store_bf16x2(sHh + (g + 8) * (CB_HC + 8) + hc, sHl + (g + 8) * (CB_HC + 8) + hc, gelu_erf_f(hacc[2] + bb0), gelu_erf_f(hacc[3] + bb1));
+    }
+    __syncthreads();
+#pragma unroll
+    for (int kk = 0; kk < CB_HC; kk += 16) {
+      unsigned ah[4], al[4];
+      ldmatrix_x4(ah, sHh + (lane & 15) * (CB_HC + 8) + kk + (lane >> 4) * 8);
+      ldmatrix_x4(al, sHl + (lane & 15) * (CB_HC + 8) + kk + (lane >> 4) * 8);
+#pragma unroll
+      for (int i = 0; i < 8; ++i) {
+        if (i < tpw && nt0 + i < ntile) {
+          unsigned bw[2];
+          ldmatrix_x2(bw, sW2 + ((nt0 + i) * 8 + (lane & 7)) * (CB_HC + 8) + kk + ((lane >> 3) & 1) * 8);
+          mma_bf16_16816(oacc[i], ah, bw[0], bw[1]);
+          mma_bf16_16816(oacc[i], al, bw[0], bw[1]);
+        }
+      }
+    }
+    __syncthreads();
+  }
+  const bool single = gridDim.y == 1;
+#pragma unroll
+  for (int i = 0; i < 8; ++i) {
+    if (i < tpw && nt0 + i < ntile) {
+#pragma unroll
+      for (int q = 0; q < 4; ++q) {
+        const int r = g + (q >> 1) * 8, nl = (nt0 + i) * 8 + q2 + (q & 1), n = col0 + nl;
+        if (r < rows) {
+          const float gm = sFg[nl];
+          float* o = p.out + ((size_t)b * T + t0 + r) * C + n;
+          if (single) *o = sX1[r * C + n] + gm * (oacc[i][q] + sB2[nl]);
+          else atomicAdd(o, gm * oacc[i][q] + (chunk == 0 ? sX1[r * C + n] + gm * sB2[nl] : 0.f));
+        }
+      }
+    }
+  }
 }
 
 struct StateSeg { float* hist; float* next; int n; };
diff --git a/vibevoice_b200/csrc/vv_runtime.cu b/vibevoice_b200/csrc/vv_runtime.cu
--- a/vibevoice_b200/csrc/vv_runtime.cu
+++ b/vibevoice_b200/csrc/vv_runtime.cu
@@ -86,8 +86,6 @@
   bf16* s_planes = nullptr; size_t planes_elems = 0;
   int mma_min_rows = 9;
   int use_wgmma = 1;
-  bool ring_rms = true;
-  int codec_mma_min_rows = 9;
   bool mma_ring = true;
   bf16* head_slab = nullptr; size_t head_slab_bytes = 0; size_t l2_persist_bytes = 0; size_t l2_window_max = 0;
   int wr_tasks_min = 296;
@@ -118,7 +116,7 @@
   int nsplit = 128;
   float *s_condp = nullptr, *s_call = nullptr, *s_mod = nullptr, *s_hx = nullptr, *s_hg = nullptr, *s_v = nullptr, *s_z = nullptr,
         *s_x0 = nullptr, *s_tfeat = nullptr, *s_t1 = nullptr, *s_hgu = nullptr;
-  float *s_xa = nullptr, *s_xb = nullptr, *s_u = nullptr, *s_win = nullptr, *s_xn = nullptr;
+  float *s_xa = nullptr, *s_xb = nullptr, *s_xc = nullptr, *s_win = nullptr;
   float *s_e = nullptr, *s_c1 = nullptr, *s_feat = nullptr, *s_audio = nullptr, *s_latent = nullptr;
   int* s_tok = nullptr;
   std::map<std::string, GraphEntry> graphs;
@@ -228,7 +226,8 @@
   }
   if (p.M >= l.c->mma_min_rows) {
     dim3 grid((p.N + MM_BN - 1) / MM_BN, (p.M + MM_BM - 1) / MM_BM);
-    const bool inplace_res = (p.epi == EPI_RESID || p.epi == EPI_GAMMA_RESID || p.epi == EPI_GATED_RESID) && p.res == p.y && p.ldres == p.ldy;
+    const bool inplace_res = ((p.epi == EPI_RESID || p.epi == EPI_GAMMA_RESID || p.epi == EPI_GATED_RESID) && p.res == p.y && p.ldres == p.ldy) ||
+                             (p.epi == EPI_NONE && p.y_zeroed);
     const int nk = (p.K + MM_BK - 1) / MM_BK;
     if (l.c->use_splitk && inplace_res && nk >= 8 && (int)(grid.x * grid.y) < l.c->sm_count) {
       int z = std::min(std::min(nk / 2, 16), (2 * l.c->sm_count) / (int)(grid.x * grid.y));
@@ -238,11 +237,8 @@
     if (l.c->mma_ring && (p.pro == PRO_NONE || ring_rms) && p.epi != EPI_SWIGLU) {
       void (*fn)(GemvP) = gemm_mma_ring_kernel<-1, -1>;
       if (!getenv("VV_RING_GENERIC")) {
-        if (ring_rms && p.epi == EPI_GELU) fn = gemm_mma_ring_kernel<1, EPI_GELU>;
-        else if (ring_rms && p.epi == EPI_NONE) fn = gemm_mma_ring_kernel<1, EPI_NONE>;
-        else if (!ring_rms && p.epi == EPI_GAMMA_RESID) fn = gemm_mma_ring_kernel<0, EPI_GAMMA_RESID>;
+        if (ring_rms && p.epi == EPI_NONE) fn = gemm_mma_ring_kernel<1, EPI_NONE>;
         else if (!ring_rms && p.epi == EPI_NONE) fn = gemm_mma_ring_kernel<0, EPI_NONE>;
-        else if (!ring_rms && p.epi == EPI_GELU) fn = gemm_mma_ring_kernel<0, EPI_GELU>;
         else if (!ring_rms && p.epi == EPI_RESID) fn = gemm_mma_ring_kernel<0, EPI_RESID>;
       }
       CK(cudaFuncSetAttribute(fn, cudaFuncAttributeMaxDynamicSharedMemorySize, MR_SMEM_NORM));
@@ -670,9 +666,6 @@
   if (getenv("VV_WGMMA")) c->use_wgmma = atoi(getenv("VV_WGMMA"));
   if (getenv("VV_MMA_MIN_ROWS")) c->mma_min_rows = atoi(getenv("VV_MMA_MIN_ROWS"));
   if (getenv("VV_NO_MMA_RING")) c->mma_ring = false;
-  if (getenv("VV_NO_RING_RMS")) c->ring_rms = false;
-  if (getenv("VV_CODEC_MMA_MIN_ROWS")) c->codec_mma_min_rows = atoi(getenv("VV_CODEC_MMA_MIN_ROWS"));
-  else if (getenv("VV_MMA_MIN_ROWS")) c->codec_mma_min_rows = c->mma_min_rows;
   const char* ns = getenv("VV_NO_SPLITK");
   c->use_splitk = !(ns && ns[0] == '1');
   const char* np = getenv("VV_NO_PDL");
@@ -1105,8 +1098,7 @@
   max_win = std::max(max_win, (size_t)(hop + 8) * 64);
   RET(dmalloc(c, &c->s_xa, (size_t)B * max_tc));
   RET(dmalloc(c, &c->s_xb, (size_t)B * max_tc));
-  RET(dmalloc(c, &c->s_xn, (size_t)B * max_tc));
-  RET(dmalloc(c, &c->s_u, (size_t)B * max_tc * 4));
+  RET(dmalloc(c, &c->s_xc, (size_t)B * max_tc));
   RET(dmalloc(c, &c->s_win, (size_t)B * max_win));
   c->planes_elems = std::max<size_t>((size_t)B * max_tc * 4, (size_t)std::max(d.max_diffusion_steps, 1) * M2 * H);
   RET(dmalloc(c, &c->s_planes, 2 * c->planes_elems));
@@ -1723,40 +1715,82 @@
   return run_cached(c, key, (cudaStream_t)stream, [&](const L& l) { return enqueue_diffusion(l, cond, noise, latent_out, sprog); });
 }
 
-static int assemble(const L& l, const float* src, const float* hist, float* win, float* next, int B, int T, int ctx, int C,
-                    const float* norm_w, float eps, float alpha, float beta) {
+static int assemble(const L& l, const float* src, const float* hist, float* win, float* next, int B, int T, int ctx, int C, float alpha, float beta,
+                    float* zero_dst = nullptr, long long zero_n = 0) {
   const int rows = B * (ctx + T);
-  if (C >= 512) CK(launch_k(l, assemble_window_block_kernel, dim3(rows), dim3(256), 0, src, hist, win, next, B, T, ctx, C, norm_w, eps, alpha, beta));
-  else CK(launch_k(l, assemble_window_kernel, dim3((rows + 7) / 8), dim3(256), 0, src, hist, win, next, B, T, ctx, C, norm_w, eps, alpha, beta));
-  return 0;
-}
-
-static int enqueue_block(const L& l, const Block& b, const float* xin, float* xout, int B, int T, float eps) {
+  if (C >= 512) CK(launch_k(l, assemble_window_block_kernel, dim3(rows), dim3(256), 0, src, hist, win, next, B, T, ctx, C, alpha, beta, zero_dst, zero_n));
+  else CK(launch_k(l, assemble_window_kernel, dim3((rows + 7) / 8), dim3(256), 0, src, hist, win, next, B, T, ctx, C, alpha, beta, zero_dst, zero_n));
+  return 0;
+}
+
+struct BlockShape { int tiles, chunks, spc, ncol, smem; };
+static BlockShape block_shape(const vv_ctx* c, int C, int T, int B) {
+  BlockShape s;
+  s.tiles = (T + CB_R - 1) / CB_R;
+  const int nsub = (4 * C + CB_HC - 1) / CB_HC;
+  for (s.ncol = std::min(C, CB_NCOL);; s.ncol /= 2) {
+    const int ctas = B * s.tiles * (C / s.ncol);
+    s.chunks = nsub;
+    for (int d = 1; d < nsub; ++d)
+      if (nsub % d == 0 && ctas * d >= c->sm_count) { s.chunks = d; break; }
+    s.spc = nsub / s.chunks;
+    s.smem = CodecBlockSmem(C, T, s.ncol, s.spc).total;
+    if (s.smem <= 227 * 1024 || s.ncol <= 64) break;
+  }
+  return s;
+}
+static int launch_block(const L& l, const Block& b, const float* x, float* out, float* zero_dst, long long zero_n, int B, int T) {
+  const int C = b.C;
+  if (C % 8 || (C > CB_NCOL && C % CB_NCOL) || (C > 16 && C < CB_KT && C != 32) || (C > CB_KT && C % CB_KT))
+    return fail(VV_ERR_INVALID, "codec block: width %d not supported", C);
+  const BlockShape s = block_shape(l.c, C, T, B);
+  CodecBlockP p;
+  p.x = x; p.out = out; p.hist = b.hist; p.next = b.next;
+  p.norm_w = b.norm_w; p.dw_w = b.dw_w; p.dw_b = b.dw_b; p.gamma = b.gamma; p.ffn_norm_w = b.ffn_norm_w; p.b1 = b.b1; p.b2 = b.b2;
+  p.ffn_gamma = b.ffn_gamma; p.w1 = b.w1; p.w2 = b.w2;
+  p.zero_dst = zero_dst; p.zero_n = zero_dst ? zero_n : 0;
+  p.T = T; p.C = C; p.tiles = s.tiles; p.spc = s.spc; p.ncol = s.ncol; p.eps = l.c->d.codec_eps;
+  if (s.smem > 227 * 1024) return fail(VV_ERR_INVALID, "codec block: %d bytes of shared memory (C=%d T=%d)", s.smem, C, T);
+  CK(cudaFuncSetAttribute(codec_block_kernel, cudaFuncAttributeMaxDynamicSharedMemorySize, 227 * 1024));
+  CK(launch_k(l, codec_block_kernel, dim3(B * s.tiles, s.chunks, C / s.ncol), dim3(256), (size_t)s.smem, p));
+  return 0;
+}
+static bool block_accumulates(const vv_ctx* c, int C, int T) { return block_shape(c, C, T, c->d.max_batch).chunks > 1; }
+
+struct TailRot {
+  float *in, *out, *spare;
+  explicit TailRot(vv_ctx* c) : in(c->s_xc), out(c->s_xb), spare(c->s_xa) {}
+  void block() { float* t = in; in = out; out = spare; spare = t; }
+  void conv() { std::swap(in, spare); }
+};
+static std::vector<std::pair<const Block*, int>> tail_blocks(const Codec& k, int first, int stop) {
+  std::vector<std::pair<const Block*, int>> v;
+  for (int i = first; i < stop; ++i)
+    for (const Block& b : k.stages[i]) v.push_back({&b, k.T[i]});
+  return v;
+}
+static int stage_blocks(const L& l, TailRot& r, const std::vector<std::pair<const Block*, int>>& blocks, size_t* next_blk, int n) {
   vv_ctx* c = l.c;
-  const int C = b.C, M = B * T;
-  RET(assemble(l, xin, b.hist, c->s_win, b.next, B, T, 6, C, b.norm_w, eps, 1.f, 0.f));
-  {
-    const long long n = (long long)M * C;
-    CK(launch_k(l, dwconv_res_kernel, dim3((unsigned)((n + 255) / 256)), dim3(256), 0, xin, c->s_win, b.dw_w, b.dw_b, b.gamma, xout, B, T, C));
-  }
-  GemvP p;
-  if (M < c->mma_min_rows || (c->ring_rms && c->mma_ring && C <= MR_MAXK_NORM && c->use_wgmma != 2)) {
-    p = mk(b.w1, b.b1, xout, C, c->s_u, 4 * C, M, 4 * C, C);
-    p.pro = PRO_RMSNORM; p.pro_w = b.ffn_norm_w; p.pro_eps = eps; p.epi = EPI_GELU;
-    RET(linear(l, p));
-  } else {
-    if (C >= 512) CK(launch_k(l, rows_norm_block_kernel, dim3(M), dim3(256), 0, xout, b.ffn_norm_w, c->s_xn, C, eps));
-    else CK(launch_k(l, rows_norm_kernel, dim3((M + 7) / 8), dim3(256), 0, xout, b.ffn_norm_w, c->s_xn, M, C, eps));
-    p = mk(b.w1, b.b1, c->s_xn, C, c->s_u, 4 * C, M, 4 * C, C);
-    p.epi = EPI_GELU;
-    RET(linear(l, p));
-  }
-  p = mk(b.w2, b.b2, c->s_u, 4 * C, xout, C, M, C, 4 * C);
-  p.epi = EPI_GAMMA_RESID; p.epi_a = b.ffn_gamma; p.res = xout; p.ldres = C;
-  return linear(l, p);
-}
-
-static int conv_apply(const L& l, const ConvL& cv, const float* win, float* y, int B, int T_out, int T_in) {
+  const int B = c->d.max_batch;
+  for (int j = 0; j < n; ++j, ++*next_blk) {
+    const auto& cur = blocks[*next_blk];
+    float* z = nullptr; long long zn = 0;
+    if (*next_blk + 1 < blocks.size()) {
+      const auto& nx = blocks[*next_blk + 1];
+      if (block_accumulates(c, nx.first->C, nx.second)) { z = r.spare; zn = (long long)B * nx.second * nx.first->C; }
+    }
+    RET(launch_block(l, *cur.first, r.in, r.out, z, zn, B, cur.second));
+    r.block();
+  }
+  return 0;
+}
+static int zero_first_block(const L& l, const std::vector<std::pair<const Block*, int>>& blocks, float* out) {
+  if (blocks.empty() || !block_accumulates(l.c, blocks[0].first->C, blocks[0].second)) return 0;
+  CK(cudaMemsetAsync(out, 0, sizeof(float) * l.c->d.max_batch * blocks[0].second * blocks[0].first->C, l.s));
+  return 0;
+}
+
+static int conv_apply(const L& l, const ConvL& cv, const float* win, float* y, int B, int T_out, int T_in, bool y_zeroed = false) {
   RowMap xm; xm.T = T_out; xm.bs = (long long)(cv.ctx + T_in) * cv.Cin; xm.rs = (long long)cv.stride * cv.Cin;
   const int M = B * T_out;
   if (cv.wf) {
@@ -1766,15 +1800,9 @@
     return 0;
   }
   GemvP p = mk(cv.w, cv.bias, win, 0, y, cv.N, M, cv.N, cv.K);
-  p.xmap = xm;
+  p.xmap = xm; p.y_zeroed = y_zeroed;
   return linear(l, p);
 }
-
-struct ScopedMinRows {
-  vv_ctx* c; int saved;
-  ScopedMinRows(vv_ctx* c_, int v) : c(c_), saved(c_->mma_min_rows) { c->mma_min_rows = v; }
-  ~ScopedMinRows() { c->mma_min_rows = saved; }
-};
 
 static bool codec_stream_stage(const vv_ctx* c, const Codec& k, int i) {
   const long long rows = (long long)c->d.max_batch * k.T[i];
@@ -1851,7 +1879,8 @@
       window_op(o, cv, cb.X[cb.cur], Tin, Tin, 1, 1.f, 0.f);
       cb.cur ^= 1;
     }
-    RET(stage_ops(b, c, cb, k.stages[i], B, k.T[i], i + 1 < nf, nullptr, 0));
+    const bool last = i + 1 == nf;
+    RET(stage_ops(b, c, cb, k.stages[i], B, k.T[i], !last, last ? TailRot(c).out : nullptr, last ? (long long)B * k.T[nf] * k.C[nf] : 0));
   }
   *out_x = c->dec_front_x = cb.X[cb.cur];
   auto it = c->sprogs.find(key);
@@ -1908,36 +1937,40 @@
 static int enqueue_decode(const L& l, const float* latent, const int32_t* active, float* audio, const vv_ctx::StreamProg* front = nullptr,
                           int n_front = 0, float* front_x = nullptr) {
   vv_ctx* c = l.c;
-  ScopedMinRows scoped(c, c->codec_mma_min_rows);
   const auto& d = c->d;
   Codec& k = c->dec;
   const int B = d.max_batch, ns = d.n_stages;
-  float *xa = c->s_xa, *xb = c->s_xb;
+  TailRot r(c);
+  const float* x = front_x;
+  if (!front) n_front = 0;
+  const auto blocks = tail_blocks(k, n_front, ns);
+  size_t next_blk = 0;
   if (front) {
     RET(launch_stream(l, *front));
-    xa = front_x;
   } else {
-    n_front = 0;
-    RET(assemble(l, latent, k.convs[0].hist, c->s_win, k.convs[0].next, B, 1, 6, 64, nullptr, 0.f, 1.0f / c->speech_scale, -c->speech_bias));
-    RET(conv_apply(l, k.convs[0], c->s_win, xa, B, 1, 1));
+    RET(zero_first_block(l, blocks, r.out));
+    RET(assemble(l, latent, k.convs[0].hist, c->s_win, k.convs[0].next, B, 1, 6, 64, 1.0f / c->speech_scale, -c->speech_bias));
+    RET(conv_apply(l, k.convs[0], c->s_win, r.spare, B, 1, 1));
+    r.conv();
+    x = r.in;
   }
   for (int i = n_front; i < ns; ++i) {
     if (i > 0) {
       const ConvL& cv = k.convs[i];
       const int Tin = k.T[i - 1];
-      RET(assemble(l, xa, cv.hist, c->s_win, cv.next, B, Tin, 1, cv.Cin, nullptr, 0.f, 1.f, 0.f));
+      RET(assemble(l, x, cv.hist, c->s_win, cv.next, B, Tin, 1, cv.Cin, 1.f, 0.f, r.spare, (long long)B * Tin * cv.N));
       RowMap xm; xm.T = Tin; xm.bs = (long long)(1 + Tin) * cv.Cin; xm.rs = cv.Cin;
-      float* dst = (xa == c->s_xa) ? c->s_xb : c->s_xa;
-      GemvP p = mk(cv.w, cv.bias, c->s_win, 0, dst, cv.N, B * Tin, cv.N, cv.K);
-      p.xmap = xm;
+      GemvP p = mk(cv.w, cv.bias, c->s_win, 0, r.spare, cv.N, B * Tin, cv.N, cv.K);
+      p.xmap = xm; p.y_zeroed = 1;
       RET(linear(l, p));
-      xa = dst; xb = (xa == c->s_xa) ? c->s_xb : c->s_xa;
+      r.conv();
     }
-    for (const Block& b : k.stages[i]) { RET(enqueue_block(l, b, xa, xb, B, k.T[i], d.codec_eps)); std::swap(xa, xb); }
+    RET(stage_blocks(l, r, blocks, &next_blk, (int)k.stages[i].size()));
+    x = r.in;
   }
   const ConvL& hd = k.convs[ns];
   const int T = k.T[ns - 1];
-  RET(assemble(l, xa, hd.hist, c->s_win, hd.next, B, T, 6, hd.Cin, nullptr, 0.f, 1.f, 0.f));
+  RET(assemble(l, x, hd.hist, c->s_win, hd.next, B, T, 6, hd.Cin, 1.f, 0.f));
   RET(conv_apply(l, hd, c->s_win, audio, B, T, T));
   CK(launch_k(l, advance_kernel, dim3(k.n_segs, B, ADV_SLICES), dim3(256), 0, k.segs_dev, active));
   return 0;
@@ -1945,40 +1978,45 @@
 
 static float* encode_front_out(vv_ctx* c, int first) {
   const Codec& k = c->enc;
-  bool in_a = true;
+  TailRot r(c);
+  r.conv();
   for (int i = 0; i < first; ++i) {
-    if (i > 0) in_a = !in_a;
-    if (k.stages[i].size() & 1) in_a = !in_a;
-  }
-  return in_a ? c->s_xa : c->s_xb;
+    if (i > 0) r.conv();
+    for (size_t j = 0; j < k.stages[i].size(); ++j) r.block();
+  }
+  return r.in;
 }
 static int enqueue_encode(const L& l, const float* audio, const int32_t* active, float* feat, const vv_ctx::StreamProg* back = nullptr) {
   vv_ctx* c = l.c;
-  ScopedMinRows scoped(c, c->codec_mma_min_rows);
   const auto& d = c->d;
   Codec& k = c->enc;
   const int B = d.max_batch, ns = d.n_stages;
   const int stop = back ? enc_back_first(c) : ns;
-  float *xa = c->s_xa, *xb = c->s_xb;
+  TailRot r(c);
+  const auto blocks = tail_blocks(k, 0, stop);
+  size_t next_blk = 0;
+  RET(zero_first_block(l, blocks, r.out));
   int hop = k.T[0];
-  RET(assemble(l, audio, k.convs[0].hist, c->s_win, k.convs[0].next, B, hop, 6, 1, nullptr, 0.f, 1.f, 0.f));
-  RET(conv_apply(l, k.convs[0], c->s_win, xa, B, hop, hop));
+  RET(assemble(l, audio, k.convs[0].hist, c->s_win, k.convs[0].next, B, hop, 6, 1, 1.f, 0.f));
+  RET(conv_apply(l, k.convs[0], c->s_win, r.spare, B, hop, hop));
+  r.conv();
   for (int i = 0; i < stop; ++i) {
     if (i > 0) {
       const ConvL& cv = k.convs[i];
       const int Tin = k.T[i - 1];
-      RET(assemble(l, xa, cv.hist, c->s_win, cv.next, B, Tin, cv.ctx, cv.Cin, nullptr, 0.f, 1.f, 0.f));
-      RET(conv_apply(l, cv, c->s_win, xb, B, k.T[i], Tin));
-      std::swap(xa, xb);
+      RET(assemble(l, r.in, cv.hist, c->s_win, cv.next, B, Tin, cv.ctx, cv.Cin, 1.f, 0.f, r.spare, (long long)B * k.T[i] * cv.N));
+      RET(conv_apply(l, cv, c->s_win, r.spare, B, k.T[i], Tin, true));
+      r.conv();
     }
-    for (const Block& b : k.stages[i]) { RET(enqueue_block(l, b, xa, xb, B, k.T[i], d.codec_eps)); std::swap(xa, xb); }
-  }
+    RET(stage_blocks(l, r, blocks, &next_blk, (int)k.stages[i].size()));
+  }
+  float* xa = r.in;
   if (back) {
     if (xa != encode_front_out(c, stop)) return fail(VV_ERR_STATE, "encoder hand-off buffer mismatch");
     RET(launch_stream(l, *back));
   } else {
     const ConvL& hd = k.convs[ns];
-    RET(assemble(l, xa, hd.hist, c->s_win, hd.next, B, 1, 6, hd.Cin, nullptr, 0.f, 1.f, 0.f));
+    RET(assemble(l, xa, hd.hist, c->s_win, hd.next, B, 1, 6, hd.Cin, 1.f, 0.f));
     RET(conv_apply(l, hd, c->s_win, feat, B, 1, 1));
   }
   CK(launch_k(l, advance_kernel, dim3(k.n_segs, B, ADV_SLICES), dim3(256), 0, k.segs_dev, active));
@@ -2087,6 +2125,22 @@
   p.pro = prologue; p.pro_w = pro_w; p.pro_eps = eps; p.epi = epilogue;
   if (epilogue == EPI_RESID) { p.res = y; p.ldres = N; }
   return linear(l, p);
+}
+
+extern "C" int vv_debug_codec_block(vv_ctx* c, int B, int T, int C, const float* norm_w, const float* dw_w, const float* dw_b, const float* gamma,
+                                    const float* ffn_norm_w, const void* w1, const float* b1, const void* w2, const float* b2, const float* ffn_gamma,
+                                    const float* x, const float* hist, float* next, float* out, void* stream) {
+  if (!c || !c->finalized) return fail(VV_ERR_STATE, "not finalized");
+  if (B < 1 || T < 1) return fail(VV_ERR_INVALID, "vv_debug_codec_block: B=%d T=%d", B, T);
+  CK(cudaSetDevice(c->device));
+  L l{c, (cudaStream_t)stream};
+  Block b;
+  b.C = C; b.norm_w = (float*)norm_w; b.dw_w = (float*)dw_w; b.dw_b = (float*)dw_b; b.gamma = (float*)gamma; b.ffn_norm_w = (float*)ffn_norm_w;
+  b.w1 = (bf16*)w1; b.b1 = (float*)b1; b.w2 = (bf16*)w2; b.b2 = (float*)b2; b.ffn_gamma = (float*)ffn_gamma; b.hist = (float*)hist; b.next = next;
+  if (block_shape(c, C, T, B).chunks > 1) CK(cudaMemsetAsync(out, 0, sizeof(float) * B * T * C, l.s));
+  RET(launch_block(l, b, x, out, nullptr, 0, B, T));
+  CK(cudaStreamSynchronize(l.s));
+  return 0;
 }
 
 static int run_debug_stream(vv_ctx* c, StreamBuilder& b, void* stream) {
```

After: 23.00, median of 6. 1.01x the previous value.
